# mpeg5/xevd

Measured on AMD Instinct MI355X. Metric: frames/sec (bit-exact YUV) + achieved HBM GB/s, higher is better.
Workload: dtype s16; 1 GPU; cfg4_main_8k_10b_ra; width=7680, height=4320, bit_depth=10, batches_resident=4, residual_pass_ahead=True, parallelism=1 stream on 1 GPU

## Files before the change

include/xevd_hip.h:

```cpp
#ifndef XEVD_HIP_H
#define XEVD_HIP_H

#include <stddef.h>
#include <stdint.h>

#ifdef __cplusplus
extern "C" {
#endif

#define XGPU_OK                    0
#define XGPU_ERR                  (-1)
#define XGPU_ERR_INVALID_ARGUMENT (-101)
#define XGPU_ERR_OUT_OF_MEMORY    (-102)
#define XGPU_ERR_UNSUPPORTED      (-104)
#define XGPU_ERR_UNEXPECTED       (-105)

#define XGPU_MAX_REFS   17
#define XGPU_PAD_L      144
#define XGPU_PAD_C      72

#define XGPU_MODE_INTRA 0
#define XGPU_MODE_INTER 1
#define XGPU_MODE_SKIP  2
#define XGPU_MODE_DIR   3
// ... 298 lines not shown
    const void *d_yuv;
    size_t size;
    int dtype;
    size_t row_pitch;
} xgpu_compare_ref;
typedef struct xgpu_compare_params {
    int crop[4];
    int ssim;
    int block_map;
} xgpu_compare_params;
typedef struct xgpu_compare_result {
    uint64_t n[3];
    uint64_t sse[3];
    uint64_t n_diff[3];
    uint64_t first_diff[3];
    uint32_t max_abs[3];
    uint32_t reserved;
    uint64_t ssim_windows[3];
    int64_t  ssim_q30[3];
} xgpu_compare_result;
size_t xgpu_compare_ref_size(const xgpu_compare_ref *r, int width, int height);
size_t xgpu_compare_map_size(const xgpu_compare_params *p, int width, int height);
int    xgpu_compare_check(const xgpu_compare_ref *r, const xgpu_compare_params *p, int width, int height, int bit_depth);
int    xgpu_pic_compare(xgpu_ctx *ctx, int pic, const xgpu_compare_ref *ref, const xgpu_compare_params *p,
                        xgpu_compare_result *d_result, uint64_t *d_map, size_t map_size, void *stream);
typedef struct xgpu_stats_params {
    int crop[4];
    int hist_bits;
    int pctl_e4[2];
    int light;
    int matrix, full_range, chroma_loc, upsample;
    int transfer;
} xgpu_stats_params;
typedef struct xgpu_stats_result {
    uint64_t n[3], sum[3], sum_sq[3];
    uint32_t min[3], max[3];
    uint32_t pctl[3][2];
    uint64_t light_n;
    double   light_sum, light_mean;
    uint32_t light_max_code, light_pctl_code[2], reserved;
    float    light_max, light_pctl[2], reserved2;
} xgpu_stats_result;
size_t xgpu_stats_hist_size(const xgpu_stats_params *p, int bit_depth);
int    xgpu_stats_check(const xgpu_stats_params *p, int width, int height, int bit_depth);
int    xgpu_stats_lin(int transfer, int bit_depth, float lin[4096]);
int    xgpu_pic_stats(xgpu_ctx *ctx, int pic, const xgpu_stats_params *p, xgpu_stats_result *d_result, uint32_t *d_hist, size_t hist_size, void *stream);
int  xgpu_pic_md5(xgpu_ctx *ctx, int pic, const xgpu_dra_luts *dra, uint8_t digest[3][16]);
int  xgpu_pic_download_padded(xgpu_ctx *ctx, int pic, int16_t *buf_y, int16_t *buf_u, int16_t *buf_v);
int  xgpu_pic_upload_padded(xgpu_ctx *ctx, int pic, const int16_t *buf_y, const int16_t *buf_u, const int16_t *buf_v);

int  xgpu_frame_begin(xgpu_ctx *ctx, const xgpu_frame_params *fp);
int  xgpu_batch_create(xgpu_ctx *ctx, const xgpu_cu_batch *b, xgpu_dbatch **out);
int  xgpu_batch_wait_upload(xgpu_ctx *ctx, xgpu_dbatch *db);
int  xgpu_batch_dmvr_mvs(xgpu_ctx *ctx, xgpu_dbatch *db, int16_t *mv, int n);
int  xgpu_set_builder_threads(xgpu_ctx *ctx, int n);
#define XGPU_BATCH_INFO_COUNT 8
int  xgpu_batch_info(xgpu_ctx *ctx, const xgpu_dbatch *db, int info[XGPU_BATCH_INFO_COUNT]);
void xgpu_batch_destroy(xgpu_ctx *ctx, xgpu_dbatch *db);
int  xgpu_batch_prepare(xgpu_ctx *ctx, xgpu_dbatch *db);
int  xgpu_batch_recon(xgpu_ctx *ctx, xgpu_dbatch *db);
int  xgpu_batch_recon_ahead(xgpu_ctx *ctx, xgpu_dbatch *db, xgpu_dbatch *next);
int  xgpu_deblock(xgpu_ctx *ctx);
int  xgpu_alf(xgpu_ctx *ctx, const xgpu_alf_params *ap);
int  xgpu_pad(xgpu_ctx *ctx);
int  xgpu_frame_end(xgpu_ctx *ctx);

enum { XGPU_K_ITDQ = 0, XGPU_K_INTER = 1, XGPU_K_DBK_V = 2, XGPU_K_DBK_H = 3, XGPU_K_PAD = 4, XGPU_K_INTRA = 5,
       XGPU_K_ALF = 6, XGPU_K_AFFINE = 7, XGPU_K_DMVR = 8, XGPU_K_COUNT = 9 };
int  xgpu_timing_enable(xgpu_ctx *ctx, int on);
int  xgpu_timing_reset(xgpu_ctx *ctx);
int  xgpu_timing_get(xgpu_ctx *ctx, double ms[XGPU_K_COUNT], long long launches[XGPU_K_COUNT]);
int  xgpu_measure_copy_bw(xgpu_ctx *ctx, size_t bytes, int iters, double *gbps);

int xgpu_test_mc_l(xgpu_ctx *ctx, const int16_t *ref_plane, int plane_w, int plane_h, int ref_x, int ref_y,
                   int has_dx, int has_dy, int gmv_x, int gmv_y, int16_t *pred, int w, int h, int bit_depth);
int xgpu_test_mc_c(xgpu_ctx *ctx, const int16_t *ref_plane, int plane_w, int plane_h, int ref_x, int ref_y,
                   int has_dx, int has_dy, int gmv_x, int gmv_y, int16_t *pred, int w, int h, int bit_depth);
int xgpu_test_recon(xgpu_ctx *ctx, const int16_t *coef, const int16_t *pred, int is_coef, int cuw, int cuh, int s_rec, int16_t *rec, int bit_depth);
int xgpu_test_dbk(xgpu_ctx *ctx, int16_t *plane, int pw, int ph, int x, int y, int st, int hor, int bit_depth);
int xgpu_test_dbk_chroma(xgpu_ctx *ctx, int16_t *u, int16_t *v, int pw, int ph, int x, int y, int st_u, int st_v, int hor, int bit_depth);
int xgpu_test_batch_resid(xgpu_ctx *ctx, xgpu_dbatch *db, int16_t *resid);
#define XGPU_TEST_BUILD_DIGESTS 13
int xgpu_test_build_batch(const xgpu_seq_params *sp, const xgpu_cu_batch *b, int threads, uint64_t digest[XGPU_TEST_BUILD_DIGESTS], int info[XGPU_BATCH_INFO_COUNT], double *ms);
int xgpu_test_itdq(xgpu_ctx *ctx, int16_t *coef, int n_blocks, int log2w, int log2h, const uint8_t *qp, int bit_depth);
int xgpu_test_itdq_ex(xgpu_ctx *ctx, int16_t *coef, int n_blocks, int log2w, int log2h, const uint8_t *qp, int bit_depth, int tr_v, int tr_h, int log2s);
int xgpu_test_itdq_pairs(xgpu_ctx *ctx, int16_t *coef, int n_blocks, int log2w, int log2h, const uint8_t *qp, int bit_depth, int tr_v, int tr_h, int log2s);
int xgpu_test_itdq_pairs_mixed(xgpu_ctx *ctx, int16_t *coef, int n_groups, const int32_t *groups, const uint8_t *qp, int bit_depth);
int xgpu_test_scale_taps_device(xgpu_ctx *ctx, int n_plane, int subsampling, int siting_half_luma, int n_dst, int filter, int32_t *first, int32_t *count,
                                int16_t *w, int w_stride);

#ifdef __cplusplus
}
#endif
#endif
```

xevd_amd/abi.py:

```python
import ctypes as C
import os

import numpy as np

HERE = os.path.dirname(os.path.abspath(__file__))
LIB_PATH = os.path.join(HERE, "libxevd_hip.so")

XGPU_MAX_REFS = 17
PAD_L, PAD_C = 144, 72
MODE_INTRA, MODE_INTER, MODE_SKIP, MODE_DIR = 0, 1, 2, 3
K_NAMES = ["itdq", "inter", "dbk_v", "dbk_h", "pad", "intra", "alf", "affine", "dmvr"]
K_COUNT = 9


class SeqParams(C.Structure):
    _fields_ = [
        ("device", C.c_int), ("width", C.c_int), ("height", C.c_int),
        ("bit_depth_luma", C.c_int), ("bit_depth_chroma", C.c_int), ("chroma_format_idc", C.c_int),
        ("log2_ctu", C.c_int), ("tool_iqt", C.c_int), ("tool_admvp", C.c_int), ("tool_addb", C.c_int),
        ("tool_alf", C.c_int), ("max_pics", C.c_int),
        ("chroma_qp_table", C.POINTER(C.c_int8) * 2),
        ("tool_eipd", C.c_int),
    ]

# ... 700 lines not shown
                                              C.c_int, C.c_void_p, C.c_size_t, C.c_void_p]),
    "xgpu_output_scaled_cm_check": (C.c_int, [C.POINTER(OutputFormat), C.POINTER(ScaleParams), C.POINTER(ColourTransform), C.c_int, C.c_int, C.c_int]),
    "xgpu_pic_output_device_scaled_cm": (C.c_int, [C.c_void_p, C.c_int, C.c_void_p, C.POINTER(OutputFormat), C.POINTER(ScaleParams), C.POINTER(ColourTransform),
                                                   C.c_void_p, C.c_size_t, C.c_void_p]),
    "xgpu_pic_output_device_rois_cm": (C.c_int, [C.c_void_p, C.c_int, C.c_void_p, C.POINTER(OutputFormat), C.POINTER(ScaleParams), C.POINTER(RoiParams), C.POINTER(Roi),
                                                 C.c_int, C.POINTER(ColourTransform), C.c_void_p, C.c_size_t, C.c_void_p]),
    "xgpu_output_scaled_lin_check": (C.c_int, [C.POINTER(OutputFormat), C.POINTER(ScaleParams), C.POINTER(ColourTransform), C.c_int, C.c_int, C.c_int]),
    "xgpu_output_rois_lin_check": (C.c_int, [C.POINTER(OutputFormat), C.POINTER(ScaleParams), C.POINTER(RoiParams), C.POINTER(Roi), C.c_int, C.POINTER(ColourTransform),
                                             C.c_int, C.c_int, C.c_int, C.POINTER(C.c_int)]),
    "xgpu_pic_output_device_scaled_lin": (C.c_int, [C.c_void_p, C.c_int, C.c_void_p, C.POINTER(OutputFormat), C.POINTER(ScaleParams), C.POINTER(ColourTransform),
                                                    C.c_void_p, C.c_size_t, C.c_void_p]),
    "xgpu_pic_output_device_rois_lin": (C.c_int, [C.c_void_p, C.c_int, C.c_void_p, C.POINTER(OutputFormat), C.POINTER(ScaleParams), C.POINTER(RoiParams), C.POINTER(Roi),
                                                  C.c_int, C.POINTER(ColourTransform), C.c_void_p, C.c_size_t, C.c_void_p]),
    "xgpu_resample_taps": (C.c_int, [C.c_int] * 6 + [C.POINTER(C.c_int32), C.POINTER(C.c_int32), C.POINTER(C.c_int16), C.c_int]),
    "xgpu_output_resampled_size": (C.c_size_t, [C.POINTER(OutputFormat), C.POINTER(ResampleParams), C.c_int, C.c_int, C.c_int]),
    "xgpu_output_resampled_check": (C.c_int, [C.POINTER(OutputFormat), C.POINTER(ResampleParams), C.c_int, C.c_int, C.c_int]),
    "xgpu_pic_output_device_resampled": (C.c_int, [C.c_void_p, C.c_int, C.c_void_p, C.POINTER(OutputFormat), C.POINTER(ResampleParams), C.c_void_p, C.c_size_t,
                                                   C.c_void_p]),
    "xgpu_output_rois_resampled_check": (C.c_int, [C.POINTER(OutputFormat), C.POINTER(ResampleParams), C.POINTER(RoiParams), C.POINTER(Roi), C.c_int, C.c_int, C.c_int,
                                                   C.c_int, C.POINTER(C.c_int)]),
    "xgpu_output_rois_resampled_size": (C.c_size_t, [C.POINTER(OutputFormat), C.POINTER(ResampleParams), C.POINTER(RoiParams), C.POINTER(Roi), C.c_int, C.c_int, C.c_int,
                                                     C.c_int]),
    "xgpu_pic_output_device_rois_resampled": (C.c_int, [C.c_void_p, C.c_int, C.c_void_p, C.POINTER(OutputFormat), C.POINTER(ResampleParams), C.POINTER(RoiParams),
                                                        C.POINTER(Roi), C.c_int, C.c_void_p, C.c_size_t, C.c_void_p]),
    "xgpu_roi_snap": (C.c_int, [C.c_int, C.c_void_p, C.c_int, C.c_int, C.POINTER(Roi)]),
    "xgpu_output_rois_dev_check": (C.c_int, [C.POINTER(OutputFormat), C.POINTER(ScaleParams), C.POINTER(RoiParams), C.POINTER(RoiBounds)] + [C.c_int] * 5),
    "xgpu_output_rois_dev_size": (C.c_size_t, [C.POINTER(OutputFormat), C.POINTER(ScaleParams), C.POINTER(RoiParams), C.POINTER(RoiBounds)] + [C.c_int] * 5),
    "xgpu_pic_output_device_rois_dev": (C.c_int, [C.c_void_p, C.c_int, C.c_void_p, C.POINTER(OutputFormat), C.POINTER(ScaleParams), C.POINTER(RoiParams),
                                                  C.POINTER(RoiBounds), C.c_int, C.c_void_p, C.c_int, C.c_void_p, C.c_void_p, C.c_void_p, C.c_size_t, C.c_void_p]),
    "xgpu_warp_from_matrix": (C.c_int, [C.POINTER(C.c_double), C.POINTER(WarpMap)]),
    "xgpu_warp_from_rotated_box": (C.c_int, [C.c_double] * 5 + [C.c_int, C.c_int, C.POINTER(WarpMap)]),
    "xgpu_output_warp_check": (C.c_int, [C.POINTER(OutputFormat), C.POINTER(ScaleParams), C.POINTER(WarpParams), C.POINTER(WarpMap), C.c_int, C.c_int, C.c_int, C.c_int,
                                         C.POINTER(C.c_int)]),
    "xgpu_output_warp_size": (C.c_size_t, [C.POINTER(OutputFormat), C.POINTER(ScaleParams), C.POINTER(WarpParams), C.c_int, C.c_int, C.c_int, C.c_int]),
    "xgpu_pic_output_device_warp": (C.c_int, [C.c_void_p, C.c_int, C.c_void_p, C.POINTER(OutputFormat), C.POINTER(ScaleParams), C.POINTER(WarpParams), C.c_void_p,
                                              C.c_int, C.c_int, C.c_void_p, C.c_void_p, C.c_size_t, C.c_void_p]),
    "xgpu_remap_grid_dims": (C.c_int, [C.c_int, C.c_int, C.c_int, C.POINTER(C.c_int), C.POINTER(C.c_int)]),
    "xgpu_remap_grid_size": (C.c_size_t, [C.POINTER(ScaleParams), C.POINTER(RemapParams), C.c_int]),
    "xgpu_output_remap_check": (C.c_int, [C.POINTER(OutputFormat), C.POINTER(ScaleParams), C.POINTER(RemapParams), C.c_int, C.c_int, C.c_int, C.c_int]),
    "xgpu_output_remap_size": (C.c_size_t, [C.POINTER(OutputFormat), C.POINTER(ScaleParams), C.POINTER(RemapParams), C.c_int, C.c_int, C.c_int, C.c_int]),
    "xgpu_remap_from_warp": (C.c_int, [C.POINTER(WarpMap), C.c_int, C.c_int, C.c_int, C.POINTER(C.c_int32)]),
    "xgpu_remap_from_homography": (C.c_int, [C.POINTER(C.c_double), C.c_int, C.c_int, C.c_int, C.POINTER(C.c_int32)]),
    "xgpu_remap_from_lens": (C.c_int, [C.POINTER(RemapLens), C.c_int, C.c_int, C.c_int, C.POINTER(C.c_int32)]),
    "xgpu_pic_output_device_remap": (C.c_int, [C.c_void_p, C.c_int, C.c_void_p, C.POINTER(OutputFormat), C.POINTER(ScaleParams), C.POINTER(RemapParams), C.c_void_p,
                                               C.c_size_t, C.c_int, C.c_void_p, C.c_size_t, C.c_void_p]),
    "xgpu_side_info_size": (C.c_size_t, [C.POINTER(SideFormat), C.c_int, C.c_int]),
    "xgpu_frame_side_info": (C.c_int, [C.c_void_p, C.c_int, C.POINTER(SideFormat), C.c_void_p, C.c_size_t, C.c_void_p]),
    "xgpu_resid_size": (C.c_size_t, [C.POINTER(ResidFormat), C.c_int, C.c_int]),
    "xgpu_batch_residual": (C.c_int, [C.c_void_p, C.c_void_p, C.POINTER(ResidFormat), C.c_void_p, C.c_size_t, C.c_void_p]),
    "xgpu_compare_ref_size": (C.c_size_t, [C.POINTER(CompareRef), C.c_int, C.c_int]),
    "xgpu_compare_map_size": (C.c_size_t, [C.POINTER(CompareParams), C.c_int, C.c_int]),
    "xgpu_compare_check": (C.c_int, [C.POINTER(CompareRef), C.POINTER(CompareParams), C.c_int, C.c_int, C.c_int]),
    "xgpu_pic_compare": (C.c_int, [C.c_void_p, C.c_int, C.POINTER(CompareRef), C.POINTER(CompareParams), C.c_void_p, C.c_void_p, C.c_size_t, C.c_void_p]),
    "xgpu_stats_hist_size": (C.c_size_t, [C.POINTER(StatsParams), C.c_int]),
    "xgpu_stats_check": (C.c_int, [C.POINTER(StatsParams), C.c_int, C.c_int, C.c_int]),
    "xgpu_stats_lin": (C.c_int, [C.c_int, C.c_int, C.POINTER(C.c_float)]),
    "xgpu_pic_stats": (C.c_int, [C.c_void_p, C.c_int, C.POINTER(StatsParams), C.c_void_p, C.c_void_p, C.c_size_t, C.c_void_p]),
    "xgpu_host_alloc": (C.c_int, [C.c_void_p, C.c_size_t, C.POINTER(C.c_void_p)]),
    "xgpu_host_free": (None, [C.c_void_p, C.c_void_p]),
    "xgpu_batch_wait_upload": (C.c_int, [C.c_void_p, C.c_void_p]),
    "xgpu_set_builder_threads": (C.c_int, [C.c_void_p, C.c_int]),
    "xgpu_batch_prepare": (C.c_int, [C.c_void_p, C.c_void_p]),
    "xgpu_batch_info": (C.c_int, [C.c_void_p, C.c_void_p, C.POINTER(C.c_int)]),
    "xgpu_batch_dmvr_mvs": (C.c_int, [C.c_void_p, C.c_void_p, C.c_void_p, C.c_int]),
    "xgpu_pic_download_padded": (C.c_int, [C.c_void_p, C.c_int, C.c_void_p, C.c_void_p, C.c_void_p]),
    "xgpu_pic_upload_padded": (C.c_int, [C.c_void_p, C.c_int, C.c_void_p, C.c_void_p, C.c_void_p]),
    "xgpu_frame_begin": (C.c_int, [C.c_void_p, C.POINTER(FrameParams)]),
    "xgpu_batch_create": (C.c_int, [C.c_void_p, C.POINTER(CuBatch), C.POINTER(C.c_void_p)]),
    "xgpu_batch_destroy": (None, [C.c_void_p, C.c_void_p]),
    "xgpu_batch_recon": (C.c_int, [C.c_void_p, C.c_void_p]),
    "xgpu_batch_recon_ahead": (C.c_int, [C.c_void_p, C.c_void_p, C.c_void_p]),
    "xgpu_deblock": (C.c_int, [C.c_void_p]),
    "xgpu_alf": (C.c_int, [C.c_void_p, C.POINTER(AlfParams)]),
    "xgpu_pad": (C.c_int, [C.c_void_p]),
    "xgpu_frame_end": (C.c_int, [C.c_void_p]),
    "xgpu_timing_enable": (C.c_int, [C.c_void_p, C.c_int]),
    "xgpu_timing_reset": (C.c_int, [C.c_void_p]),
    "xgpu_timing_get": (C.c_int, [C.c_void_p, C.POINTER(C.c_double), C.POINTER(C.c_longlong)]),
    "xgpu_measure_copy_bw": (C.c_int, [C.c_void_p, C.c_size_t, C.c_int, C.POINTER(C.c_double)]),
    "xgpu_test_mc_l": (C.c_int, [C.c_void_p, C.c_void_p] + [C.c_int] * 8 + [C.c_void_p] + [C.c_int] * 3),
    "xgpu_test_mc_c": (C.c_int, [C.c_void_p, C.c_void_p] + [C.c_int] * 8 + [C.c_void_p] + [C.c_int] * 3),
    "xgpu_test_batch_resid": (C.c_int, [C.c_void_p, C.c_void_p, C.c_void_p]),
    "xgpu_test_build_batch": (C.c_int, [C.c_void_p, C.c_void_p, C.c_int, C.POINTER(C.c_uint64), C.POINTER(C.c_int), C.POINTER(C.c_double)]),
    "xgpu_test_recon": (C.c_int, [C.c_void_p, C.c_void_p, C.c_void_p] + [C.c_int] * 4 + [C.c_void_p, C.c_int]),
    "xgpu_test_dbk": (C.c_int, [C.c_void_p, C.c_void_p] + [C.c_int] * 7),
    "xgpu_test_dbk_chroma": (C.c_int, [C.c_void_p, C.c_void_p, C.c_void_p] + [C.c_int] * 8),
    "xgpu_test_itdq": (C.c_int, [C.c_void_p, C.c_void_p, C.c_int, C.c_int, C.c_int, C.c_void_p, C.c_int]),
    "xgpu_test_itdq_ex": (C.c_int, [C.c_void_p, C.c_void_p, C.c_int, C.c_int, C.c_int, C.c_void_p, C.c_int, C.c_int, C.c_int, C.c_int]),
    "xgpu_test_itdq_pairs": (C.c_int, [C.c_void_p, C.c_void_p, C.c_int, C.c_int, C.c_int, C.c_void_p, C.c_int, C.c_int, C.c_int, C.c_int]),
    "xgpu_test_itdq_pairs_mixed": (C.c_int, [C.c_void_p, C.c_void_p, C.c_int, C.c_void_p, C.c_void_p, C.c_int]),
    "xgpu_test_scale_taps_device": (C.c_int, [C.c_void_p] + [C.c_int] * 5 + [C.POINTER(C.c_int32), C.POINTER(C.c_int32), C.POINTER(C.c_int16), C.c_int]),
}

_lib = None


def exported_names():
    return sorted(_EXPORTS)


def _share_torch_hip_runtime():
    import importlib.util
    import sys
    if "torch" in sys.modules:
        return
    spec = importlib.util.find_spec("torch")
    if spec is None or not spec.submodule_search_locations:
        return
    rt = os.path.join(list(spec.submodule_search_locations)[0], "lib", "libamdhip64.so")
    if os.path.exists(rt):
        C.CDLL(rt, mode=C.RTLD_GLOBAL)


def load():
    global _lib
    if _lib is None:
        _share_torch_hip_runtime()
        if not os.path.exists(LIB_PATH):
            raise RuntimeError(
                f"{LIB_PATH} is missing: build it with `python -c 'import __graft_entry__ as g; g.build()'` "
                "(hipcc --offload-arch=gfx950).  xevd_amd has no CPU fallback.")
        lib = C.CDLL(LIB_PATH)
        for name, (res, args) in _EXPORTS.items():
            fn = getattr(lib, name)
            fn.restype, fn.argtypes = res, args
        _lib = lib
    return _lib
```

xevd_amd/csrc/k_alf.hip:

```cpp
#include "xgpu_internal.h"
#include "addb_filter.h"

typedef short v2s __attribute__((ext_vector_type(2)));

#define LROWS 72
#define LSTR  72
#define CROWS 36
#define CSTR  40

struct CtuRect { int x0, y0, cw, ch, aL, aR, aT, aB; int tx0, tx1, ty0, ty1; };

__device__ __forceinline__ void alf_pos(const CtuRect k, int y, int x, int &yy, int &xx)
{
    yy = y; xx = x;
    if (y < k.y0 && !k.aT) yy = 2 * k.y0 - y;
    else if (y >= k.y0 + k.ch && !k.aB) yy = 2 * (k.y0 + k.ch - 1) - y;
    if (yy >= k.y0 && yy < k.y0 + k.ch) {
        if (x < k.x0 && !k.aL) xx = 2 * k.x0 - x;
        else if (x >= k.x0 + k.cw && !k.aR) xx = 2 * (k.x0 + k.cw - 1) - x;
    }
    yy = min(max(yy, k.ty0), k.ty1 - 1); xx = min(max(xx, k.tx0), k.tx1 - 1);
}
__device__ __forceinline__ int alf_fetch(const int16_t *__restrict__ p, int s, const CtuRect k, int y, int x)
{
// ... 25 lines not shown
        } else if (ty0 + r < k.y0 + k.ch + H && tx0 + c4 < k.x0 + k.cw + H) {
#pragma unroll
            for (int e = 0; e < 4; e++) lds[(r + H) * STR + c4 + e + OFF] = (int16_t)alf_fetch(p, s, k, ty0 + r, tx0 + c4 + e);
        }
    }
    constexpr int RING = (T + 2 * H) * (T + 2 * H) - T * T;
    for (int i = t0; i < RING; i += nthr) {
        int r, c;
        if (i < H * (T + 2 * H)) { r = i / (T + 2 * H) - H; c = i % (T + 2 * H) - H; }
        else if (i < 2 * H * (T + 2 * H)) { const int j = i - H * (T + 2 * H); r = T + j / (T + 2 * H); c = j % (T + 2 * H) - H; }
        else { const int j = i - 2 * H * (T + 2 * H); r = j / (2 * H); const int q = j % (2 * H); c = q < H ? q - H : T + q - H; }
        lds[(r + H) * STR + c + OFF] = (int16_t)alf_fetch(p, s, k, ty0 + r, tx0 + c);
    }
}

__device__ __forceinline__ v2s asv(uint32_t x) { return __builtin_bit_cast(v2s, x); }
__device__ __forceinline__ uint32_t asu(v2s x) { return __builtin_bit_cast(uint32_t, x); }
__device__ __forceinline__ v2s vabs(v2s x) { const v2s z = {0, 0}; const v2s n = z - x; return __builtin_elementwise_max(x, n); }
__device__ __forceinline__ int mad_lo(uint32_t ps, int f, int acc) { int r; asm("v_mad_i32_i16 %0, %1, %2, %3" : "=v"(r) : "v"(ps), "v"(f), "v"(acc)); return r; }
__device__ __forceinline__ int mad_hi(uint32_t ps, int f, int acc) { int r; asm("v_mad_i32_i16 %0, %1, %2, %3 op_sel:[1,0,0,0]" : "=v"(r) : "v"(ps), "v"(f), "v"(acc)); return r; }
__device__ __forceinline__ int mad_lo_fh(uint32_t ps, uint32_t f, int acc) { int r; asm("v_mad_i32_i16 %0, %1, %2, %3 op_sel:[0,1,0,0]" : "=v"(r) : "v"(ps), "v"(f), "v"(acc)); return r; }
__device__ __forceinline__ int mad_hi_fh(uint32_t ps, uint32_t f, int acc) { int r; asm("v_mad_i32_i16 %0, %1, %2, %3 op_sel:[1,1,0,0]" : "=v"(r) : "v"(ps), "v"(f), "v"(acc)); return r; }
#define SC_ "s"
__device__ __forceinline__ int smad_lo(uint32_t ps, uint32_t f, int acc) { int r; asm("v_mad_i32_i16 %0, %1, %2, %3" : "=v"(r) : "v"(ps), SC_(f), "v"(acc)); return r; }
__device__ __forceinline__ int smad_hi(uint32_t ps, uint32_t f, int acc) { int r; asm("v_mad_i32_i16 %0, %1, %2, %3 op_sel:[1,0,0,0]" : "=v"(r) : "v"(ps), SC_(f), "v"(acc)); return r; }
__device__ __forceinline__ int smad_lo_fh(uint32_t ps, uint32_t f, int acc) { int r; asm("v_mad_i32_i16 %0, %1, %2, %3 op_sel:[0,1,0,0]" : "=v"(r) : "v"(ps), SC_(f), "v"(acc)); return r; }
__device__ __forceinline__ int smad_hi_fh(uint32_t ps, uint32_t f, int acc) { int r; asm("v_mad_i32_i16 %0, %1, %2, %3 op_sel:[1,1,0,0]" : "=v"(r) : "v"(ps), SC_(f), "v"(acc)); return r; }
__device__ __forceinline__ int dot2s_first(uint32_t f, uint32_t x) { int r; asm("v_dot2_i32_i16 %0, %1, %2, %3" : "=v"(r) : "v"(f), "v"(x), SC_(256)); return r; }
__device__ __forceinline__ int sdot2s(uint32_t f, uint32_t x, int acc) { int r; asm("v_dot2_i32_i16 %0, %1, %2, %3" : "=v"(r) : SC_(f), "v"(x), "v"(acc)); return r; }
__device__ __forceinline__ uint32_t clip_pack(int o0, int o1, int maxv)
{
    int a, b;
    asm("v_med3_i32 %0, %1, 0, %2" : "=v"(a) : "v"(o0 >> 9), SC_(maxv));
    asm("v_med3_i32 %0, %1, 0, %2" : "=v"(b) : "v"(o1 >> 9), SC_(maxv));
    return __builtin_amdgcn_perm((uint32_t)b, (uint32_t)a, 0x05040100u);
}
typedef unsigned short v2us __attribute__((ext_vector_type(2)));
__device__ __forceinline__ uint32_t padd(uint32_t x, uint32_t y) { return __builtin_bit_cast(uint32_t, __builtin_bit_cast(v2us, x) + __builtin_bit_cast(v2us, y)); }
__device__ __forceinline__ uint32_t padd_x(uint32_t x, uint32_t y) { uint32_t r; asm("v_pk_add_u16 %0, %1, %2 op_sel:[0,1] op_sel_hi:[1,0]" : "=v"(r) : "v"(x), "v"(y)); return r; }
__device__ __forceinline__ uint32_t pack_f(int lo, int hi) { return ((uint32_t)lo & 0xFFFFu) | ((uint32_t)hi << 16); }
__device__ __forceinline__ int dot2s(uint32_t f, uint32_t x, int acc) { return __builtin_amdgcn_sdot2(__builtin_bit_cast(v2s, f), __builtin_bit_cast(v2s, x), acc, false); }
__device__ __forceinline__ void lap_pair(const uint32_t up[3], const uint32_t mid[3], const uint32_t dn[3], uint32_t acc[4])
{
    const uint32_t c2 = padd(mid[1], mid[1]);
    const uint32_t l0 = __builtin_amdgcn_alignbit(mid[1], mid[0], 16), r0 = __builtin_amdgcn_alignbit(mid[2], mid[1], 16);
    const uint32_t lu = __builtin_amdgcn_alignbit(up[1], up[0], 16), ru = __builtin_amdgcn_alignbit(up[2], up[1], 16);
    const uint32_t ld = __builtin_amdgcn_alignbit(dn[1], dn[0], 16), rd = __builtin_amdgcn_alignbit(dn[2], dn[1], 16);
    acc[0] = __builtin_amdgcn_sad_u16(c2, padd(up[1], dn[1]), acc[0]);
    acc[1] = __builtin_amdgcn_sad_u16(c2, padd(l0, r0), acc[1]);
    acc[2] = __builtin_amdgcn_sad_u16(c2, padd(lu, rd), acc[2]);
    acc[3] = __builtin_amdgcn_sad_u16(c2, padd(ld, ru), acc[3]);
}

#ifdef XGPU_ALF_TRACE
__device__ unsigned long long g_alf_trace[16];
#define ATR(p) do { if (atr_on) { const unsigned long long now_ = __builtin_amdgcn_s_memtime(); atomicAdd(&g_alf_trace[p], now_ - atr_prev); atr_prev = __builtin_amdgcn_s_memtime(); } } while (0)
extern "C" int xgpu_test_alf_trace(unsigned long long out[16], int reset)
{
    if (hipMemcpyFromSymbol(out, HIP_SYMBOL(g_alf_trace), sizeof(g_alf_trace)) != hipSuccess) return -1;
    if (reset) { static unsigned long long z[16]; if (hipMemcpyToSymbol(HIP_SYMBOL(g_alf_trace), z, sizeof(z)) != hipSuccess) return -1; }
    return 0;
}
#else
#define ATR(p) do { } while (0)
#endif
#ifndef XGPU_ALF_WAVES
#define XGPU_ALF_WAVES 6
#endif
template <bool FUSED, bool PK = false>
__device__ __forceinline__ void alf_kernel(const AlfArgs &a, const AddbArgs *d, const int16_t *__restrict__ sy_, const int16_t *__restrict__ su_,
                                           const int16_t *__restrict__ sv_, int16_t *__restrict__ dy_, int16_t *__restrict__ du_,
                                           int16_t *__restrict__ dv_)
{
    constexpr int RO = FUSED ? 4 : 3, CO = FUSED ? 2 : 4;
    __shared__ __attribute__((aligned(16))) int16_t l_y[LROWS * LSTR];
    __shared__ __attribute__((aligned(16))) int16_t l_c[2][CROWS * CSTR];
    constexpr int LAP_BYTES = 7168;
    static_assert(17 * 17 * 16 <= LAP_BYTES, "the offset-lattice sums fit");
    __shared__ __attribute__((aligned(16))) uint8_t l_lap[LAP_BYTES];
    uint4 (*const l_o)[17] = (uint4 (*)[17])l_lap;
    int16_t (*b_row)[2][64] = (int16_t (*)[2][64])l_y, (*b_col)[2][64] = (int16_t (*)[2][64])(l_y + 3 * 2 * 64);
    static_assert(2 * 3 * 2 * 64 <= LROWS * LSTR, "the border arrays fit into the staged luma tile");

    const int tiles_x = (a.pic_w + 63) >> 6, n_tiles = tiles_x * ((a.pic_h + 63) >> 6);
    const int per_xcd = gridDim.x >> 3, xcd = blockIdx.x & 7, seq = blockIdx.x >> 3;
    const int tile = xcd * per_xcd + (xcd >= 4 ? per_xcd - 1 - seq : seq);
    if (tile >= n_tiles) return;
    const int ty = a.magic_tiles_x ? (int)__umulhi((uint32_t)tile, a.magic_tiles_x) : tile, tx = tile - ty * tiles_x;
    const int tx0 = tx << 6, ty0 = ty << 6;
    const int t = threadIdx.x;
#ifdef XGPU_ALF_TRACE
    unsigned long long atr_prev = __builtin_amdgcn_s_memtime();
    const bool atr_on = (t & 63) == 0 && tile % 61 == 7;
    if (atr_on) atomicAdd(&g_alf_trace[15], 1ull);
#endif
    CtuRect k, kc;
    bool luma_on;
    auto ctu_setup = [&]() {
    const int ctu = 1 << a.log2_ctu;
    k.x0 = tx0 & ~(ctu - 1); k.y0 = ty0 & ~(ctu - 1);
    k.cw = min(ctu, a.pic_w - k.x0); k.ch = min(ctu, a.pic_h - k.y0);
    k.tx0 = 0; k.tx1 = a.pic_w; k.ty0 = 0; k.ty1 = a.pic_h;
    if (a.multi_tile) {
        const int cx = k.x0 >> a.log2_ctu, cy = k.y0 >> a.log2_ctu, h_ctu = (a.pic_h + ctu - 1) >> a.log2_ctu;
        k.tx0 = TileMask::tile_first(a.tiles.vb, cx) << a.log2_ctu; k.tx1 = min(TileMask::tile_end(a.tiles.vb, cx, a.w_ctu) << a.log2_ctu, a.pic_w);
        k.ty0 = TileMask::tile_first(a.tiles.hb, cy) << a.log2_ctu; k.ty1 = min(TileMask::tile_end(a.tiles.hb, cy, h_ctu) << a.log2_ctu, a.pic_h);
    }
    k.aL = a.across_tiles ? k.x0 != 0 : k.x0 != k.tx0; k.aT = a.across_tiles ? k.y0 != 0 : k.y0 != k.ty0;
    k.aR = a.across_tiles ? 1 : (k.x0 + k.cw != k.tx1);
    k.aB = a.across_tiles ? 1 : (k.y0 + k.ch != k.ty1);
    const int ctu_idx = (k.y0 >> a.log2_ctu) * a.w_ctu + (k.x0 >> a.log2_ctu);
    luma_on = a.enable[0] && (a.ctb_in_args ? ((a.ctb_bits[ctu_idx >> 5] >> (ctu_idx & 31)) & 1) != 0 : (a.ctb_flag == nullptr || a.ctb_flag[ctu_idx] != 0));
    kc = k;
    kc.x0 >>= 1; kc.y0 >>= 1; kc.cw >>= 1; kc.ch >>= 1; kc.tx0 >>= 1; kc.tx1 >>= 1; kc.ty0 >>= 1; kc.ty1 >>= 1;
    };
    if (!FUSED) ctu_setup();
    if (!FUSED) {
        if (luma_on) alf_stage<64, 3, LSTR, 4>(l_y, sy_, a.s_l, k, tx0, ty0, t, 256);
        if (a.enable[1]) alf_stage<32, 2, CSTR, 4>(l_c[0], su_, a.s_c, kc, tx0 >> 1, ty0 >> 1, t, 256);
        if (a.enable[2]) alf_stage<32, 2, CSTR, 4>(l_c[1], sv_, a.s_c, kc, tx0 >> 1, ty0 >> 1, t, 256);
        __syncthreads();
    } else {
        const AddbArgs &da = *d;
        uint4 (*s_map)[18] = (uint4 (*)[18])l_lap;
        uint8_t *s_alpha = (uint8_t *)l_lap + 18 * 18 * 16, *s_beta = s_alpha + 52, *s_clip = s_beta + 52, *s_pic = s_clip + 260;
        int8_t *s_cqp = (int8_t *)(s_pic + XGPU_MAX_REFS * 2);
        static_assert(52 + 52 + 260 + XGPU_MAX_REFS * 2 + 192 == ADDB_LDS_TABLE_BYTES, "the LDS tables are AddbArgs.lds_tables");
        constexpr int LIST_OFF = (18 * 18 * 16 + ADDB_LDS_TABLE_BYTES + 3) & ~3;
        uint32_t *s_cnt = (uint32_t *)((uint8_t *)l_lap + LIST_OFF);
        uint32_t (*s_list)[164] = (uint32_t (*)[164])(s_cnt + 2);
        TileMask *s_tm = (TileMask *)((uint8_t *)l_lap + LIST_OFF + 8 + 2 * 164 * 4);
        static_assert(LIST_OFF + 8 + 2 * 164 * 4 + (int)sizeof(TileMask) <= LAP_BYTES, "the deblocking state fits into l_lap");
#define PK2(lo, hi) ((uint32_t)(uint16_t)(lo) | ((uint32_t)(uint16_t)(hi) << 16))
        const bool interior = tx0 > 0 && ty0 > 0 && tx0 + 68 <= a.pic_w && ty0 + 68 <= a.pic_h;
        if (interior) {
            const int wave = __builtin_amdgcn_readfirstlane(t >> 6);
            typedef __attribute__((address_space(3))) char lds_char;
            typedef const __attribute__((address_space(1))) char glb_char;
            {
                const int r0 = (t * 57) >> 9, c0 = t - r0 * 9;
                glb_char *const g0 = (glb_char *)(sy_ + (ty0 - 4) * a.s_l + tx0 - 4);
                lds_char *const d0 = (lds_char *)l_y + wave * 1024;
                const uint32_t rs = (uint32_t)a.s_l << 1;
                const int c1 = c0 + 4 >= 9 ? c0 - 5 : c0 + 4, r1 = r0 + 28 + (c0 + 4 >= 9), c2 = c0 + 8 >= 9 ? c0 - 1 : c0 + 8, r2 = r0 + 56 + (c0 + 8 >= 9);
                __builtin_amdgcn_global_load_lds((glb_char *)(g0 + r0 * rs + c0 * 16), (lds_char *)d0, 16, 0, 0);
                __builtin_amdgcn_global_load_lds((glb_char *)(g0 + r1 * rs + c1 * 16), (lds_char *)(d0 + 4096), 16, 0, 0);
                if (t < 648 - 512) __builtin_amdgcn_global_load_lds((glb_char *)(g0 + r2 * rs + c2 * 16), (lds_char *)(d0 + 8192), 16, 0, 0);
            }
            {
                const uint32_t rs = (uint32_t)a.s_c << 1;
                const uint32_t cbase = (uint32_t)(((ty0 >> 1) - 2) * a.s_c + (tx0 >> 1) - 2) << 1;
                lds_char *const d0 = (lds_char *)&l_c[0][0] + wave * 1024;
#pragma unroll
                for (int it = 0; it < 2; it++) {
                    const int idx = t + 256 * it, pl = idx >= 180, j = idx - 180 * pl, r = (j * 205) >> 10, c = j - r * 5;
                    if (it == 0 || t < 360 - 256)
                        __builtin_amdgcn_global_load_lds((glb_char *)((glb_char *)(pl ? sv_ : su_) + cbase + r * rs + c * 16), (lds_char *)(d0 + 4096 * it), 16, 0, 0);
                }
            }
            {
                glb_char *const g0 = (glb_char *)(da.maps + ((ty0 >> 2) - 1) * da.w_scu + (tx0 >> 2) - 1);
                lds_char *const d0 = (lds_char *)l_lap + wave * 1024;
                const uint32_t rs = (uint32_t)da.w_scu << 4;
#pragma unroll
                for (int it = 0; it < 2; it++) {
                    const int idx = t + 256 * it, r = (idx * 57) >> 10, c = idx - r * 18;
                    if (it == 0 || t < 324 - 256) __builtin_amdgcn_global_load_lds((glb_char *)(g0 + r * rs + c * 16), (lds_char *)(d0 + 4096 * it), 16, 0, 0);
                }
            }
            __builtin_amdgcn_sched_barrier(0);
            {
                static_assert(ADDB_LDS_TABLE_DWORDS + 16 <= 256, "one table dword per thread");
                if (t < ADDB_LDS_TABLE_DWORDS) ((uint32_t *)s_alpha)[t] = da.lds_tables[t];
                else if (t < ADDB_LDS_TABLE_DWORDS + 16) { const int k_ = t - ADDB_LDS_TABLE_DWORDS; ((uint32_t *)s_tm)[k_] = k_ < 8 ? da.no_filter.vb[k_] : da.no_filter.hb[k_ - 8]; }
                if (t < 2) s_cnt[t] = 0;
            }
// ... 347 lines not shown
        if (!a.enable[1 + pl]) {
#pragma unroll
            for (int ii = 0; ii < 2; ii++) {
                const uint32_t w = FUSED ? *(const uint32_t *)(l_c[pl] + ((ly << 1) + ii + 2) * CSTR + (lx << 1) + CO) : *(const uint32_t *)(src + (cy + ii) * a.s_c + cx);
                *(uint32_t *)((char *)dst + (oc0 + ii * sc2)) = w; keep_chroma(ii, w);
            }
            continue;
        }
        uint32_t C[6][3];
#pragma unroll
        for (int i = 0; i < 6; i++) {
            const uint32_t *row = (const uint32_t *)(l_c[pl] + ((ly << 1) + i) * CSTR + (lx << 1) + CO - 2);
            C[i][0] = row[0]; C[i][1] = row[1]; C[i][2] = row[2];
        }
#define PC(i, c) ((((c) + 2) & 1) ? __builtin_amdgcn_alignbit(C[(i) + 2][(((c) + 2) >> 1) + 1], C[(i) + 2][((c) + 2) >> 1], 16) : C[(i) + 2][((c) + 2) >> 1])
        const uint32_t G32 = a.cchroma[0], G54 = a.cchroma[1], G10 = a.cchroma[2], G6 = a.cchroma[3];
        const uint32_t G32v = G32;
#pragma unroll
        for (int ii = 0; ii < 2; ii++) {
            int o[2];
#pragma unroll
            for (int jj = 0; jj < 2; jj++) {
                int acc = sdot2s(G54, padd_x(PC(ii, jj + 1), PC(ii, jj - 2)), dot2s_first(G32v, padd_x(PC(ii + 1, jj - 1), PC(ii - 1, jj))));
                o[jj] = smad_lo(PC(ii, jj), G6, acc);
            }
            const uint32_t p0 = padd(PC(ii + 2, 0), PC(ii - 2, 0)), p1 = padd(PC(ii + 1, 1), PC(ii - 1, -1));
            o[0] = smad_lo_fh(p1, G10, smad_lo(p0, G10, o[0]));
            o[1] = smad_hi_fh(p1, G10, smad_hi(p0, G10, o[1]));
            const uint32_t w = clip_pack(o[0], o[1], maxv);
            *(uint32_t *)((char *)dst + (oc0 + ii * sc2)) = w;
            keep_chroma(ii, w);
        }
#undef PC
    }
    } while (0);

    ATR(11);
    if (!a.pad || !(edge_l || edge_r || edge_t || edge_b)) return;
    __syncthreads();
#pragma unroll
    for (int c = 0; c < 3; c++) {
        const int sh = c ? 1 : 0, pad = c ? XGPU_PAD_C : XGPU_PAD_L, s = c ? a.s_c : a.s_l;
        const int pw = a.pic_w >> sh, ph = a.pic_h >> sh, x0 = tx0 >> sh, y0 = ty0 >> sh, T = 64 >> sh;
        const int cols = min(T, pw - x0), rows = min(T, ph - y0);
        int16_t *pl = c == 0 ? dy_ : (c == 1 ? du_ : dv_);
        const int q = pad >> 2;
#pragma unroll
        for (int side = 0; side < 2; side++) {
            if (side ? !edge_r : !edge_l) continue;
            for (int i = t; i < rows * q; i += 256) {
                const int r = i / q, k = i - r * q;
                const uint32_t v = (uint16_t)b_col[c][side][r] * 0x10001u;
                *(uint2 *)(pl + (y0 + r) * s + (side ? pw : -pad) + 4 * k) = make_uint2(v, v);
            }
        }
#pragma unroll
        for (int side = 0; side < 2; side++) {
            if (side ? !edge_b : !edge_t) continue;
            int16_t *base = pl + (side ? ph : -pad) * s;
            const int cq = cols >> 2;
            for (int i = t; i < pad * cq; i += 256) {
                const int r = i / cq, k = i - r * cq;
                *(uint2 *)(base + r * s + x0 + 4 * k) = *(const uint2 *)&b_row[c][side][4 * k];
            }
#pragma unroll
            for (int cs = 0; cs < 2; cs++) {
                if (cs ? !edge_r : !edge_l) continue;
                const uint32_t v = (uint16_t)b_row[c][side][cs ? cols - 1 : 0] * 0x10001u;
                for (int i = t; i < pad * q; i += 256) {
                    const int r = i / q, k = i - r * q;
                    *(uint2 *)(base + r * s + (cs ? pw : -pad) + 4 * k) = make_uint2(v, v);
                }
            }
        }
    }
}

__global__ __launch_bounds__(256) void k_alf(const AlfArgs a, const int16_t *__restrict__ sy_, const int16_t *__restrict__ su_, const int16_t *__restrict__ sv_,
                                             int16_t *__restrict__ dy_, int16_t *__restrict__ du_, int16_t *__restrict__ dv_)
{
    alf_kernel<false>(a, nullptr, sy_, su_, sv_, dy_, du_, dv_);
}

template <bool PK>
__global__ __launch_bounds__(256) __attribute__((amdgpu_waves_per_eu(XGPU_ALF_WAVES, XGPU_ALF_WAVES))) void k_addb_alf(const AlfArgs a, const AddbArgs d, const int16_t *__restrict__ sy_, const int16_t *__restrict__ su_,
                                                  const int16_t *__restrict__ sv_, int16_t *__restrict__ dy_, int16_t *__restrict__ du_, int16_t *__restrict__ dv_)
{
    alf_kernel<true, PK>(a, &d, sy_, su_, sv_, dy_, du_, dv_);
}

void launch_alf(xgpu_ctx *c, const AlfArgs &a_, const AddbArgs *deblock, const DevPic &src, const DevPic &dst)
{
    AlfArgs a = a_;
    const int tiles = ((a.pic_w + 63) >> 6) * ((a.pic_h + 63) >> 6);
    a.magic_tiles_x = a.pic_w > 64 ? (uint32_t)((1ull << 32) / (uint64_t)((a.pic_w + 63) >> 6)) + 1u : 0u;
    const dim3 grid(((tiles + 7) >> 3) << 3);
    const bool scalar_knob = c->addb_scalar != 0;
    static const int lds_pad = getenv("XEVD_HIP_ALF_LDSPAD") ? atoi(getenv("XEVD_HIP_ALF_LDSPAD")) : 0;
    if (deblock && !scalar_knob && deblock->bd_l <= 10 && deblock->bd_c <= 10) hipLaunchKernelGGL(k_addb_alf<true>, grid, dim3(256), lds_pad, c->stream, a, *deblock, src.y, src.u, src.v, dst.y, dst.u, dst.v);
    else if (deblock) hipLaunchKernelGGL(k_addb_alf<false>, grid, dim3(256), 0, c->stream, a, *deblock, src.y, src.u, src.v, dst.y, dst.u, dst.v);
    else hipLaunchKernelGGL(k_alf, grid, dim3(256), 0, c->stream, a, src.y, src.u, src.v, dst.y, dst.u, dst.v);
}
```

xevd_amd/csrc/k_inter.hip:

```cpp
#include "xgpu_internal.h"

#include <hip/hip_ext.h>
#include <type_traits>
#include "mc_filters.h"

#define LDS_AS __attribute__((address_space(3)))

#define UW_STRIDE 48
#define UI_STRIDE 40
#define UC_STRIDE 24
#define UCW_STRIDE 32
static_assert(UI_STRIDE <= UW_STRIDE && UC_STRIDE <= UCW_STRIDE, "an intermediate row is not longer than the window row it replaces");
#define UT_L_SAMPLES (40 * UW_STRIDE)
#define UT_C_SAMPLES (3 * 64 * 8)
#define UNI_SAMPLES   (UT_L_SAMPLES + UT_C_SAMPLES)
static_assert(2 * 19 * UCW_STRIDE <= UT_C_SAMPLES, "both chroma windows fit");

__device__ __forceinline__ void wave_lds_sync()
{
    __builtin_amdgcn_fence(__ATOMIC_RELEASE, "wavefront");
    __builtin_amdgcn_wave_barrier();
    __builtin_amdgcn_fence(__ATOMIC_ACQUIRE, "wavefront");
}

// ... 548 lines not shown
            }
            TRACE_MARK(tr, 6);
            {
                const uint2 th = s_ctap[cdx ? ((px & 7) << 2) : 32], tv = s_ctap[cdy ? ((py & 7) << 2) : 32];
                const uint32_t c2h[2] = { th.x, th.y }, c2v[2] = { tv.x, tv.y };
                const Regime rg = regime(cdx, cdy, a.bd_c);
                const int mis = ((px >> 3) - 1) & 7, odd = mis & 1;
                const int16_t *const Wu = Wu0 + (mis & ~1), *const Wv = Wu + C_SAMPLES;
                if (cdx) { if (cdy) chroma_tile_filter<true, true, WS_C, true>(Wu, Wv, c2h, c2v, rg, maxc, IC, lane, ou, ov, odd); else chroma_tile_filter<true, false, WS_C, true>(Wu, Wv, c2h, c2v, rg, maxc, IC, lane, ou, ov, odd); }
                else     { if (cdy) chroma_tile_filter<false, true, WS_C, true>(Wu, Wv, c2h, c2v, rg, maxc, IC, lane, ou, ov, odd); else chroma_tile_filter<false, false, WS_C, true>(Wu, Wv, c2h, c2v, rg, maxc, IC, lane, ou, ov, odd); }
            }
            TRACE_MARK(tr, 7);
            if (more) {
                if (REGION) __syncthreads(); else wave_lds_sync();
                request_chroma(1);
            }
            if (nl == 0) {
#pragma unroll
                for (int k = 0; k < 8; k++) pl[k] = o[k];
                pu[0] = ou[0]; pu[1] = ou[1]; pv[0] = ov[0]; pv[1] = ov[1];
            } else {
#pragma unroll
                for (int k = 0; k < 8; k++) pl[k] = avg2(pl[k], o[k]);
                pu[0] = avg2(pu[0], ou[0]); pu[1] = avg2(pu[1], ou[1]);
                pv[0] = avg2(pv[0], ov[0]); pv[1] = avg2(pv[1], ov[1]);
            }
            nl++;
        }
        (void)tid;
    } else {
        TRACE_MARK(tr, 2);
#pragma unroll
        for (int l = 0; l < 2; l++) {
            if (!use[l]) continue;
            const uint4 e0 = s_ref[refis[l] * 2 + l][0], e1 = s_ref[refis[l] * 2 + l][1];
            const gs16 ry_ = (gs16)(((uint64_t)e0.y << 32) | e0.x), ru_ = (gs16)(((uint64_t)e0.w << 32) | e0.z), rv_ = (gs16)(((uint64_t)e1.y << 32) | e1.x);
            const int mvx = mvs[l][0], mvy = mvs[l][1];
            const int px = (x << 2) + mvt[l][0], py = (y << 2) + mvt[l][1];
            const int ldx = (mvx & 3) != 0, ldy = (mvy & 3) != 0;
            const int cdx = (mvx & 7) != 0, cdy = (mvy & 7) != 0;
            uint32_t ch[4], cv[4], o[8], ou[2], ov[2];
            {
                const uint4 th = s_ltap[ldx ? ((px & 3) << 2) : 16], tv = s_ltap[ldy ? ((py & 3) << 2) : 16];
                ch[0] = th.x; ch[1] = th.y; ch[2] = th.z; ch[3] = th.w; cv[0] = tv.x; cv[1] = tv.y; cv[2] = tv.z; cv[3] = tv.w;
                const uint2 cth = s_ctap[cdx ? ((px & 7) << 2) : 32], ctv = s_ctap[cdy ? ((py & 7) << 2) : 32];
                const uint32_t c2h[2] = { cth.x, cth.y }, c2v[2] = { ctv.x, ctv.y };
                const gs16 p = ry_ + ((py >> 2) - 3) * a.s_l + (px >> 2) - 3;
                const int off = ((py >> 3) - 1) * a.s_c + (px >> 3) - 1;
                const Regime rgl = regime(ldx, ldy, a.bd_l), rgc = regime(cdx, cdy, a.bd_c);
                const bool wh = __ballot(ldx) != 0, wvv = __ballot(ldy) != 0;
                const bool cwh = __ballot(cdx) != 0, cwv = __ballot(cdy) != 0;
#define MC_S(H, V) mc_scu_list<H, V>(p, a.s_l, ru_ + off, rv_ + off, a.s_c, ch, cv, rgl, maxl, c2h, c2v, rgc, maxc, cwh, cwv, o, ou, ov, ldx != 0, ldy != 0, cdx != 0, cdy != 0)
                if (wh) { if (wvv) MC_S(true, true); else MC_S(true, false); }
                else    { if (wvv) MC_S(false, true); else MC_S(false, false); }
#undef MC_S
            }
            if (nl == 0) {
#pragma unroll
                for (int k = 0; k < 8; k++) pl[k] = o[k];
                pu[0] = ou[0]; pu[1] = ou[1]; pv[0] = ov[0]; pv[1] = ov[1];
            } else {
#pragma unroll
                for (int k = 0; k < 8; k++) pl[k] = avg2(pl[k], o[k]);
                pu[0] = avg2(pu[0], ou[0]); pu[1] = avg2(pu[1], ou[1]);
                pv[0] = avg2(pv[0], ov[0]); pv[1] = avg2(pv[1], ov[1]);
            }
            nl++;
        }
    }
    TRACE_MARK(tr, 9);
    if (MODE == 0) load_resid();
    if (nl == 0) return false;

    if (cbf & 1) {
#pragma unroll
        for (int k = 0; k < 8; k++) pl[k] = recon2(pl[k], rl[k], maxl);
    }
    if (cbf & 2) { pu[0] = recon2(pu[0], ru[0], maxl); pu[1] = recon2(pu[1], ru[1], maxl); }
    if (cbf & 4) { pv[0] = recon2(pv[0], rv[0], maxl); pv[1] = recon2(pv[1], rv[1], maxl); }

    return true;
}

__device__ __forceinline__ int xcd_slice(int block, int grid) { return (block & 7) * (grid >> 3) + (block >> 3); }

__device__ __forceinline__ void store_scu(const InterArgs &a, int sx, int sy, const uint32_t pl[8], const uint32_t pu[2], const uint32_t pv[2])
{
    const int x = sx << 2, y = sy << 2;
    int16_t *dy = a.cur_y + y * a.s_l + x;
#pragma unroll
    for (int k = 0; k < 4; k++) *(uint2 *)(dy + k * a.s_l) = make_uint2(pl[k * 2], pl[k * 2 + 1]);
    const int coff = (y >> 1) * a.s_c + (x >> 1);
    *(uint32_t *)(a.cur_u + coff) = pu[0];
    *(uint32_t *)(a.cur_u + coff + a.s_c) = pu[1];
    *(uint32_t *)(a.cur_v + coff) = pv[0];
    *(uint32_t *)(a.cur_v + coff + a.s_c) = pv[1];
}
#define ARG_REFS(a)  ((const uint4 (*)[2])&(a).refp[0][0])
#define ARG_LTAPS(a) ((const uint4 *)&k_luma_taps[(a).admvp][0][0])
#define ARG_CTAPS(a) ((const uint2 *)&k_chroma_taps[(a).admvp][0][0])
static_assert(sizeof(RefEntry) == 32, "a reference entry is two 16-byte halves");
static_assert(XGPU_INTER_STRIP == 16, "the strip arithmetic below shifts by four");

struct SplitTables { uint4 ref[XGPU_MAX_REFS * 2][2]; uint4 ltap[17]; uint2 ctap[33]; uint2 pad; };

__device__ __forceinline__ void inter_fused_body(const InterArgs &a)
{
    __shared__ __attribute__((aligned(16))) int16_t s_win[REG_SAMPLES];
    static_assert(4 * UNI_SAMPLES <= REG_SAMPLES, "the four waves' tile blocks fit into the region block");
    __shared__ SplitTables s_tab[4];
    const int idx = xcd_slice(blockIdx.x, gridDim.x);
    if (idx >= a.n_work) return;
    const int t = threadIdx.x, lane = t & 63, wave = __builtin_amdgcn_readfirstlane(t >> 6);
#ifdef XGPU_INTER_TRACE
    InterTrace tr = { __builtin_amdgcn_s_memtime(), 0, lane == 0 && (idx % 61) == 7 };
#endif
    int rx, ry;
    if (idx < a.full_entries) {
        const int s = (int)__umulhi((uint32_t)idx, a.magic_strip), r = idx - s * a.strip_entries;
        ry = r >> 4; rx = (s << 4) + (r & 15);
    } else {
        const int r = idx - a.full_entries;
        ry = a.magic_last ? (int)__umulhi((uint32_t)r, a.magic_last) : r; rx = (a.regions_x & ~15) + r - ry * (a.regions_x & 15);
    }
    const int sx = (rx << 4) + ((wave & 1) << 3) + (lane & 7), sy = (ry << 4) + ((wave >> 1) << 3) + (lane >> 3);
    const uint32_t kinds = a.work[idx];
    const uint4 *const item = (const uint4 *)&a.items[idx * 4 + wave];
    const uint4 e = item[0], i0 = item[1], i1 = item[2];
    const uint32_t own = (sx < (a.pic_w >> 2) && sy < (a.pic_h >> 2)) ? a.owner[sy * a.w_scu + sx] : OWNER_NONE;
    const LaneMap fm0 = { 0, 0 };
    uint32_t pl[8], pu[2], pv[2];
    if (kinds == XGPU_WORK_REGION) {
#ifdef XGPU_INTER_TRACE
        tr.role = 0;
        if (e.y == 0xFFFFFFFFu) tr.on = false;
        if (tr.on) atomicAdd(&g_inter_trace[0][15], 1ull);
        TRACE_MARK(tr, 0);
#endif
        const RegionMap rmap = region_map(t);
        if (inter_tile<2>(a, i0, i1, true, sx, sy, lane, s_win, fm0, ARG_REFS(a), ARG_LTAPS(a), ARG_CTAPS(a), pl, pu, pv, &rmap, wave, e.y TRACE_PASS)) store_scu(a, sx, sy, pl, pu, pv);
        TRACE_MARK(tr, 10);
        return;
    }
    const uint32_t kind = (kinds >> (2 * wave)) & 3u;
    if (kind == 1) {
#ifdef XGPU_INTER_TRACE
        tr.role = 1;
        if (e.y == 0xFFFFFFFFu) tr.on = false;
        if (tr.on) atomicAdd(&g_inter_trace[1][15], 1ull);
        TRACE_MARK(tr, 0);
#endif
        LaneMap fm;
        {
            const int row0 = (lane * 171) >> 10, k = lane - row0 * 6;
            fm.gy = row0 * a.s_l + 8 * k; fm.ly = row0 * UW_STRIDE + 8 * k;
        }
        if (inter_tile<1>(a, i0, i1, true, sx, sy, lane, s_win + wave * UNI_SAMPLES, fm, ARG_REFS(a), ARG_LTAPS(a), ARG_CTAPS(a), pl, pu, pv, nullptr, 0, e.y TRACE_PASS)) store_scu(a, sx, sy, pl, pu, pv);
        TRACE_MARK(tr, 10);
    } else if (kind == 2) {
#ifdef XGPU_INTER_TRACE
        tr.role = 2;
        if (tr.on) atomicAdd(&g_inter_trace[2][15], 1ull);
        TRACE_MARK(tr, 0);
#endif
        SplitTables &tb = s_tab[wave];
        static_assert(XGPU_MAX_REFS * 4 == 68, "lanes 0..63 and 0..3 of the second round take the reference entries' halves");
        const uint4 tab0 = ((const uint4 *)&a.refp[0][0])[lane];
        uint4 tab1 = make_uint4(0, 0, 0, 0);
        if (lane < 4) tab1 = ((const uint4 *)&a.refp[0][0])[64 + lane];
        else if (lane < 4 + 17) tab1 = *(const uint4 *)k_luma_taps[a.admvp][lane - 4];
        else if (lane < 4 + 17 + 33) { const uint2 v = *(const uint2 *)k_chroma_taps[a.admvp][lane - 21]; tab1.x = v.x; tab1.y = v.y; }
        const bool ok = own < (uint32_t)a.n_cu;
        uint4 c0 = make_uint4(0, 0, 0, 0), c1 = c0;
        if (ok) { c0 = ((const uint4 *)&a.cus[own])[0]; c1 = ((const uint4 *)&a.cus[own])[1]; }
        tb.ref[lane >> 1][lane & 1] = tab0;
        if (lane < 4) tb.ref[32 + (lane >> 1)][lane & 1] = tab1;
        else if (lane < 4 + 17) tb.ltap[lane - 4] = tab1;
        else if (lane < 4 + 17 + 33) tb.ctap[lane - 21] = make_uint2(tab1.x, tab1.y);
        wave_lds_sync();
        TRACE_MARK(tr, 1);
        if (inter_tile<0>(a, c0, c1, ok, sx, sy, lane, nullptr, fm0, tb.ref, tb.ltap, tb.ctap, pl, pu, pv, nullptr, 0, own TRACE_PASS)) store_scu(a, sx, sy, pl, pu, pv);
        TRACE_MARK(tr, 10);
    }
}
__global__ __launch_bounds__(256) void k_inter(const InterArgs a) { inter_fused_body(a); }

void launch_inter(xgpu_ctx *c, const InterArgs &a)
{
    if (!a.n_work) return;
    const dim3 grid((unsigned)(((a.n_work + 7) >> 3) << 3));
    hipLaunchKernelGGL(k_inter, grid, dim3(256), 0, c->stream, a);
}

__global__ void k_test_mc(const int16_t *plane, int stride, int ref_x, int ref_y, int has_dx, int has_dy, int gmv_x, int gmv_y,
                          int16_t *pred, int w, int h, int bd, int luma, int admvp)
{
    const int bs = luma ? 4 : 2;
    const int nbx = w / bs, nby = h / bs;
    const int i = blockIdx.x * blockDim.x + threadIdx.x;
    if (i >= nbx * nby) return;
    const int bx = (i % nbx) * bs, by = (i / nbx) * bs;
    const int maxv = (1 << bd) - 1;
    const int16_t *ref = plane + ref_y * stride + ref_x;
    if (luma) {
        const uint32_t *th = k_luma_taps[admvp][has_dx ? (gmv_x & 15) : 16], *tv = k_luma_taps[admvp][has_dy ? (gmv_y & 15) : 16];
        uint32_t ch[4] = { th[0], th[1], th[2], th[3] }, cv[4] = { tv[0], tv[1], tv[2], tv[3] }, o[8];
        const gs16 p = (gs16)ref + ((gmv_y >> 4) - 3 + by) * stride + (gmv_x >> 4) - 3 + bx;
        if (has_dx) { if (has_dy) mc_luma_4x4<true, true>(p, stride, ch, cv, regime(has_dx, has_dy, bd), maxv, o); else mc_luma_4x4<true, false>(p, stride, ch, cv, regime(has_dx, has_dy, bd), maxv, o); }
        else        { if (has_dy) mc_luma_4x4<false, true>(p, stride, ch, cv, regime(has_dx, has_dy, bd), maxv, o); else mc_luma_4x4<false, false>(p, stride, ch, cv, regime(has_dx, has_dy, bd), maxv, o); }
        for (int r = 0; r < 4; r++) {
            *(uint32_t *)(pred + (by + r) * w + bx) = o[r * 2];
            *(uint32_t *)(pred + (by + r) * w + bx + 2) = o[r * 2 + 1];
        }
    } else {
        const uint32_t *th = k_chroma_taps[admvp][has_dx ? (gmv_x & 31) : 32], *tv = k_chroma_taps[admvp][has_dy ? (gmv_y & 31) : 32];
        uint32_t ch[2] = { th[0], th[1] }, cv[2] = { tv[0], tv[1] }, o[2];
        const gs16 p = (gs16)ref + ((gmv_y >> 5) - 1 + by) * stride + (gmv_x >> 5) - 1 + bx;
        if (has_dx) { if (has_dy) mc_chroma_2x2<true, true>(p, stride, ch, cv, regime(has_dx, has_dy, bd), maxv, o); else mc_chroma_2x2<true, false>(p, stride, ch, cv, regime(has_dx, has_dy, bd), maxv, o); }
        else        { if (has_dy) mc_chroma_2x2<false, true>(p, stride, ch, cv, regime(has_dx, has_dy, bd), maxv, o); else mc_chroma_2x2<false, false>(p, stride, ch, cv, regime(has_dx, has_dy, bd), maxv, o); }
        *(uint32_t *)(pred + by * w + bx) = o[0];
        *(uint32_t *)(pred + (by + 1) * w + bx) = o[1];
    }
}

void launch_test_mc(xgpu_ctx *c, const int16_t *plane, int stride, int ref_x, int ref_y, int has_dx, int has_dy,
                    int gmv_x, int gmv_y, int16_t *pred, int w, int h, int bd, int luma)
{
    const int bs = luma ? 4 : 2;
    const int n = (w / bs) * (h / bs);
    hipLaunchKernelGGL(k_test_mc, dim3((n + 63) / 64), dim3(64), 0, c->stream, plane, stride, ref_x, ref_y, has_dx, has_dy,
                       gmv_x, gmv_y, pred, w, h, bd, luma, c->sp.tool_admvp);
}

__global__ void k_test_recon(const int16_t *coef, const int16_t *pred, int is_coef, int cuw, int cuh, int16_t *rec, int s_rec, int bd)
{
    const int i = blockIdx.x * blockDim.x + threadIdx.x, pw = cuw >> 1;
    if (i >= pw * cuh) return;
    const int y = i / pw, x = (i - y * pw) * 2;
    const uint32_t p = *(const uint32_t *)(pred + y * cuw + x);
    const uint32_t r = recon2(p, is_coef ? *(const uint32_t *)(coef + y * cuw + x) : 0u, (1 << bd) - 1);
    rec[y * s_rec + x] = (int16_t)(r & 0xFFFF); rec[y * s_rec + x + 1] = (int16_t)(r >> 16);
}
void launch_test_recon(xgpu_ctx *c, const int16_t *coef, const int16_t *pred, int is_coef, int cuw, int cuh, int16_t *rec, int s_rec, int bd)
{
    const int n = (cuw >> 1) * cuh;
    hipLaunchKernelGGL(k_test_recon, dim3((n + 63) / 64), dim3(64), 0, c->stream, coef, pred, is_coef, cuw, cuh, rec, s_rec, bd);
}
```

xevd_amd/csrc/xgpu_api.hip:

```cpp
#include "xgpu_host.h"

static const int8_t k_chroma_qp_main[58] = { 0, 1, 2, 3, 4, 5, 6, 7, 8, 9, 10, 11, 12, 13, 14, 15, 16, 17, 18, 19, 20, 21, 22, 23, 24, 25, 26, 27, 28, 29,
    29, 30, 31, 32, 33, 34, 35, 36, 37, 37, 38, 39, 40, 40, 41, 42, 43, 44, 45, 46, 47, 48, 49, 50, 51, 52, 53, 54 };
static const int8_t k_chroma_qp_base[58] = {
     0,  1,  2,  3,  4,  5,  6,  7,  8,  9, 10, 11, 12, 13, 14, 15, 16, 17, 18, 19,
    20, 21, 22, 23, 24, 25, 26, 27, 28, 29, 29, 29, 30, 31, 32, 32, 33, 33, 34, 34,
    35, 35, 36, 36, 36, 37, 37, 37, 38, 38, 39, 39, 40, 40, 40, 41, 41, 41 };


const char *xgpu_version(void) { return "xevd_amd 0.1 (gfx950)"; }
const char *xgpu_last_error(const xgpu_ctx *c) { return c ? c->err : "null ctx"; }

void time_begin(xgpu_ctx *c, int k, hipEvent_t *a, hipEvent_t *b)
{
    if (!c->timing) return;
    auto get = [&]() {
        hipEvent_t e;
        if (!c->ev_pool.empty()) { e = c->ev_pool.back(); c->ev_pool.pop_back(); }
        else (void)hipEventCreate(&e);
        return e;
    };
    *a = get(); *b = get();
    (void)hipEventRecord(*a, c->stream);
    (void)k;
// ... 6 lines not shown
}
int xgpu_timing_enable(xgpu_ctx *c, int on) { ARGCHK(c, c != NULL); c->timing = on; return XGPU_OK; }
int xgpu_timing_reset(xgpu_ctx *c)
{
    ARGCHK(c, c != NULL);
    HIPCHK(c, hipStreamSynchronize(c->stream));
    for (auto &e : c->ev_pending) { c->ev_pool.push_back(e.a); c->ev_pool.push_back(e.b); }
    c->ev_pending.clear();
    memset(c->t_ms, 0, sizeof(c->t_ms));
    memset(c->t_n, 0, sizeof(c->t_n));
    return XGPU_OK;
}
int xgpu_timing_get(xgpu_ctx *c, double ms[XGPU_K_COUNT], long long n[XGPU_K_COUNT])
{
    ARGCHK(c, c != NULL);
    HIPCHK(c, hipStreamSynchronize(c->stream));
    for (auto &e : c->ev_pending) {
        float t = 0;
        HIPCHK(c, hipEventElapsedTime(&t, e.a, e.b));
        c->t_ms[e.k] += t; c->t_n[e.k]++;
        c->ev_pool.push_back(e.a); c->ev_pool.push_back(e.b);
    }
    c->ev_pending.clear();
    for (int i = 0; i < XGPU_K_COUNT; i++) { ms[i] = c->t_ms[i]; n[i] = c->t_n[i]; }
    return XGPU_OK;
}

static void init_transform_tables(xgpu_ctx *c)
{
    static int tm[5460];
    int o = 0;
    for (int l = 1; l <= 6; l++) {
        const int N = 1 << l;
        for (int k = 0; k < N; k++)
            for (int n = 0; n < N; n++) {
                const double v = k == 0 ? 64.0 : 64.0 * sqrt(2.0) * cos((2 * n + 1) * k * 3.14159265358979323846 / (2.0 * N));
                tm[o++] = (int)(v >= 0 ? floor(v + 0.5) : -floor(-v + 0.5));
            }
    }
    static int16_t ats[2 * 1360];
    for (int t = 0; t < 2; t++) {
        int q = t * 1360;
        for (int l = 2; l <= 5; l++) {
            const int N = 1 << l;
            const double sc = sqrt((double)N) * 64;
            int16_t m[32 * 32];
            for (int k = 0; k < N; k++)
                for (int n = 0; n < N; n++) {
                    const double v = t == 0 ? sin(3.14159265358979323846 * (k + 0.5) * (n + 1) / (N + 0.5)) * sqrt(2.0 / (N + 0.5))
                                            : cos(3.14159265358979323846 * (k + 0.5) * (n + 0.5) / (N + 0.5)) * sqrt(2.0 / (N + 0.5));
                    m[k * N + n] = (int16_t)(sc * v + (v > 0 ? 0.5 : -0.5));
                }
            if (N == 4) {
                const int a = m[0], b = m[1], cc = m[2], d = m[3];
                const int e7[16] = { a, b, cc, b + a,  cc, cc, 0, -cc,  a + b, -a, -cc, b,  b, -(b + a), cc, -a };
                const int e8[16] = { d + cc, b, cc, d,  b, 0, -b, -b,  cc, -b, -d, d + cc,  d, -b, d + cc, -cc };
                for (int i = 0; i < 16; i++) m[i] = (int16_t)(t == 0 ? e7[i] : e8[i]);
            }
            for (int i = 0; i < N * N; i++) ats[q++] = m[i];
        }
    }
    upload_transform_tables(tm, ats, c->stream);
}

int xgpu_open(const xgpu_seq_params *sp, xgpu_ctx **out)
{
    if (!sp || !out) return XGPU_ERR_INVALID_ARGUMENT;
    *out = NULL;
    if (sp->chroma_format_idc != 1) return XGPU_ERR_UNSUPPORTED;
    if (sp->width <= 0 || sp->height <= 0 || (sp->width & 7) || (sp->height & 7)) return XGPU_ERR_INVALID_ARGUMENT;
    if (sp->bit_depth_luma < 8 || sp->bit_depth_luma > 12 || sp->bit_depth_chroma < 8 || sp->bit_depth_chroma > 12) return XGPU_ERR_UNSUPPORTED;
    if (sp->log2_ctu < 5 || sp->log2_ctu > 7) return XGPU_ERR_INVALID_ARGUMENT;
    int ndev = 0;
    if (hipGetDeviceCount(&ndev) != hipSuccess || ndev <= 0 || sp->device < 0 || sp->device >= ndev) return XGPU_ERR_UNEXPECTED;

    xgpu_ctx *c = new xgpu_ctx();
    c->sp = *sp;
    c->sp.chroma_qp_table[0] = c->sp.chroma_qp_table[1] = NULL;
    c->builder_threads = 1;
    c->err[0] = 0; c->timing = 0; c->have_frame = 0; c->side_pic = -1; c->d_maps = NULL; c->d_dra = NULL; c->d_cm = NULL; c->cm_tab = NULL; c->d_ctb_flag = NULL; c->stream = 0; c->up_stream = 0; c->down_stream = 0; c->side_stream = 0; c->after_inter = 0; c->have_after_inter = 0; c->where = 0; c->addb_pending = 0;
    c->fork_ev = c->join_ev = 0;
    c->itdq_pair_min = getenv("XEVD_HIP_ITDQ_PAIR_MIN") ? std::max(1, atoi(getenv("XEVD_HIP_ITDQ_PAIR_MIN"))) : 4096;
    c->intra_small_min = getenv("XEVD_HIP_INTRA_SMALL_MIN") ? std::max(1, atoi(getenv("XEVD_HIP_INTRA_SMALL_MIN"))) : 2048;
    c->addb_scalar = getenv("XEVD_HIP_ADDB_SCALAR") != NULL;
    c->dmvr_scalar = getenv("XEVD_HIP_DMVR_SCALAR") != NULL;
    c->split_addb_alf = getenv("XEVD_HIP_SPLIT_ADDB_ALF") != NULL;
    for (int i = 0; i < 2; i++) { c->d_out[i] = NULL; c->out_caps[i] = 0; c->out_ready[i] = c->out_done[i] = 0; c->out_busy[i] = 0; }
    c->d_md5 = NULL; c->md5_ready = 0;
    c->odev_ev[0] = c->odev_ev[1] = 0;
    c->sc_tab = NULL; c->sc_tab_cap = 0; c->sc_mid = NULL; c->sc_mid_cap = 0; c->cmp_part = NULL; c->cmp_part_cap = 0; c->stats_blk = NULL; c->stats_lin_tc = c->stats_lin_bd = -1;
    c->roi_blk = NULL; c->roi_blk_cap = 0;
    c->rs_blk = NULL; c->rs_blk_cap = 0; c->rs_key[0] = -1; c->rs_capy = c->rs_capc = 0;
    c->lad_blk = NULL; c->lad_blk_cap = 0; c->lad_cap = 0;
    for (int i = 0; i < 6; i++) c->sc_key[i] = -1;
    c->out_next = 0;
    memset(c->t_ms, 0, sizeof(c->t_ms)); memset(c->t_n, 0, sizeof(c->t_n));
    const int boff = 6 * (sp->bit_depth_chroma - 8);
    for (int t = 0; t < 2; t++)
        for (int q = -boff; q <= 57; q++)
            c->chroma_qp[t][q + boff] = sp->chroma_qp_table[t] ? sp->chroma_qp_table[t][q + boff] : (int8_t)(q < 0 ? q : (sp->tool_iqt ? k_chroma_qp_main[q] : k_chroma_qp_base[q]));

    auto fail = [&](int code) { xgpu_close(c); return code; };
    if (hipSetDevice(sp->device) != hipSuccess) return fail(XGPU_ERR_UNEXPECTED);
    static const bool blocking = getenv("XEVD_HIP_BLOCKING_SYNC") != NULL && atoi(getenv("XEVD_HIP_BLOCKING_SYNC")) != 0;
    if (blocking) (void)hipSetDeviceFlags(hipDeviceScheduleBlockingSync);
    const unsigned ev_flags = hipEventDisableTiming | (blocking ? hipEventBlockingSync : 0);
    {
        static std::atomic<int> n_ctx(0);
        static const bool no_rot = getenv("XEVD_HIP_NO_QUEUE_ROTATION") != NULL;
        const bool swap = !no_rot && (n_ctx.fetch_add(1) & 1);
        hipStream_t *const order[4] = { swap ? &c->side_stream : &c->stream, &c->up_stream, &c->down_stream, swap ? &c->stream : &c->side_stream };
        for (int i = 0; i < 4; i++)
            if (hipStreamCreateWithFlags(order[i], hipStreamNonBlocking) != hipSuccess) return fail(XGPU_ERR_UNEXPECTED);
    }
    if (hipEventCreateWithFlags(&c->after_inter, hipEventDisableTiming) != hipSuccess) return fail(XGPU_ERR_UNEXPECTED);
    if (hipEventCreateWithFlags(&c->fork_ev, hipEventDisableTiming) != hipSuccess || hipEventCreateWithFlags(&c->join_ev, hipEventDisableTiming) != hipSuccess) return fail(XGPU_ERR_UNEXPECTED);
    for (int i = 0; i < 2; i++)
        if (hipEventCreateWithFlags(&c->out_ready[i], hipEventDisableTiming) != hipSuccess || hipEventCreateWithFlags(&c->out_done[i], ev_flags) != hipSuccess)
            return fail(XGPU_ERR_UNEXPECTED);

    ctx_geometry(c);

    if (hipMalloc((void **)&c->d_maps, sizeof(ScuRec) * (size_t)c->w_scu * c->h_scu) != hipSuccess) return fail(XGPU_ERR_OUT_OF_MEMORY);
    if (hipMemsetAsync(c->d_maps, 0, sizeof(ScuRec) * (size_t)c->w_scu * c->h_scu, c->stream) != hipSuccess) return fail(XGPU_ERR_UNEXPECTED);
    if (hipMalloc((void **)&c->d_ctb_flag, (size_t)c->w_ctu * c->h_ctu + 16) != hipSuccess) return fail(XGPU_ERR_OUT_OF_MEMORY);
    init_transform_tables(c);
    c->pics.resize(1 + std::max(1, std::min(sp->max_pics, 34)));
    for (auto &p : c->pics) { p.base = NULL; p.used = 0; }
    {
        DevPic &p = c->pics[0];
        if (hipMalloc((void **)&p.base, c->pic_elems * sizeof(int16_t)) != hipSuccess) return fail(XGPU_ERR_OUT_OF_MEMORY);
        (void)hipMemsetAsync(p.base, 0, c->pic_elems * sizeof(int16_t), c->stream);
        p.s_l = c->s_l; p.s_c = c->s_c; p.used = 1;
        p.y = p.base + (size_t)XGPU_PAD_L * c->s_l + XGPU_MARGIN_L;
        p.u = p.base + c->off_u + (size_t)XGPU_PAD_C * c->s_c + XGPU_MARGIN_C;
        p.v = p.base + c->off_v + (size_t)XGPU_PAD_C * c->s_c + XGPU_MARGIN_C;
    }
    if (hipStreamSynchronize(c->stream) != hipSuccess) return fail(XGPU_ERR_UNEXPECTED);
    *out = c;
    return XGPU_OK;
}

void xgpu_close(xgpu_ctx *c)
{
    if (!c) return;
    (void)hipSetDevice(c->sp.device);
    if (c->stream) (void)hipStreamSynchronize(c->stream);
    if (c->up_stream) (void)hipStreamSynchronize(c->up_stream);
    if (c->down_stream) (void)hipStreamSynchronize(c->down_stream);
    if (c->side_stream) (void)hipStreamSynchronize(c->side_stream);
    for (auto &p : c->pics) if (p.base) (void)hipFree(p.base);
    if (c->d_maps) (void)hipFree(c->d_maps);
    for (BatchBlock &k : c->pool) block_free(k);
    for (auto &h : c->pinned) (void)hipHostFree(h.p);
    c->pinned.clear();
    c->pool.clear();
    if (c->d_md5) (void)hipFree(c->d_md5);
    if (c->md5_ready) (void)hipEventDestroy(c->md5_ready);
    for (int i = 0; i < 2; i++) if (c->odev_ev[i]) (void)hipEventDestroy(c->odev_ev[i]);
    for (int i = 0; i < 2; i++) { if (c->d_out[i]) (void)hipFree(c->d_out[i]); if (c->out_ready[i]) (void)hipEventDestroy(c->out_ready[i]); if (c->out_done[i]) (void)hipEventDestroy(c->out_done[i]); }
    if (c->d_dra) (void)hipFree(c->d_dra);
    if (c->d_cm) (void)hipFree(c->d_cm);
    delete c->cm_tab;
    if (c->sc_tab) (void)hipFree(c->sc_tab);
    if (c->sc_mid) (void)hipFree(c->sc_mid);
    if (c->cmp_part) (void)hipFree(c->cmp_part);
// ... 241 lines not shown
```

xevd_amd/csrc/xgpu_builder.hip:

```cpp
#include <chrono>
#include "xgpu_host.h"
#include "affine_model.h"

namespace {
enum Seg { SEG_CUS, SEG_CTU, SEG_TBS, SEG_WAVES, SEG_INTRA, SEG_DEPS, SEG_AFF, SEG_CPMV, SEG_DMVR, SEG_OWNER, SEG_IITEM, SEG_IWORK, SEG_COEF, SEG_RESID, SEG_DONE, SEG_DMV, SEG_COUNT };
struct StageLayout {
    size_t off[SEG_COUNT], alloc[SEG_COUNT], payload[SEG_COUNT], stage_bytes, d_need;
    template <class T> T *at(void *base, Seg s) const { return (T *)((uint8_t *)base + off[s]); }
};
struct SegSize { Seg seg; size_t elem, count, min_count; };
template <size_t N> void stage_layout(StageLayout &L, const SegSize (&rows)[N])
{
    static_assert(N == SEG_COUNT, "one row per segment");
    size_t o = 0;
    for (const SegSize &r : rows) {
        L.off[r.seg] = o; L.payload[r.seg] = r.elem * r.count; L.alloc[r.seg] = r.elem * std::max(r.count, r.min_count);
        if (r.seg == SEG_COEF) L.stage_bytes = o + L.alloc[r.seg];
        o += (L.alloc[r.seg] + 255) / 256 * 256;
    }
    L.d_need = o;
}
enum { NCLS = 64 * 9 };
inline int ats_inter_of(const xgpu_cu_batch *b, int i) { return (b->ats_inter && b->pred_mode[i] != XGPU_MODE_INTRA && b->pred_mode[i] != XGPU_MODE_IBC) ? b->ats_inter[i] : 0; }
inline int tr_code(const xgpu_cu_batch *b, int i, int k)
{
    if (k != 0) return 0;
    if (const int ai = ats_inter_of(b, i)) {
        if (b->log2w[i] > 5 || b->log2h[i] > 5) return 0;
        const int idx = ai & 15, pos = ai >> 4, hor = idx == 2 || idx == 4;
        const int tv = hor ? (pos == 0 ? TR_DCT8 : TR_DST7) : TR_DST7, th = hor ? TR_DST7 : (pos == 0 ? TR_DCT8 : TR_DST7);
        return tv * 3 + th;
    }
    if (!b->ats || !(b->ats[i] & 1) || b->pred_mode[i] != XGPU_MODE_INTRA) return 0;
    const int tv = (b->ats[i] >> 1) & 1 ? TR_DCT8 : TR_DST7, th = (b->ats[i] >> 2) & 1 ? TR_DCT8 : TR_DST7;
    return tv * 3 + th;
}
template <class F> inline size_t for_each_tb(const xgpu_cu_batch *b, int i, F &&f)
{
    int bw = b->log2w[i], bh = b->log2h[i]; const int idx = ats_inter_of(b, i) & 15;
    if (idx == 1 || idx == 3) bw -= idx == 3 ? 2 : 1;
    if (idx == 2 || idx == 4) bh -= idx == 4 ? 2 : 1;
    const int nsx = b->log2w[i] > 6 ? 2 : 1, nsy = b->log2h[i] > 6 ? 2 : 1;
    size_t ext = 0;
    for (int k = 0; k < 3; k++) {
        if (!((b->cbf[i] >> k) & 1)) continue;
        const int cl = k ? bw - 1 : bw, ch = k ? bh - 1 : bh;
        const int tw = std::min(bw, 6) - (k ? 1 : 0), th = std::min(bh, 6) - (k ? 1 : 0), cls = tr_code(b, i, k) * 64 + tw * 8 + th;
        for (int sb = 0; sb < 4; sb++) {
            if ((sb & 1) >= nsx || (sb >> 1) >= nsy) continue;
            if (nsx * nsy > 1 && b->cbf_sub && !((b->cbf_sub[i] >> (4 * k + sb)) & 1)) continue;
            f(k, sb, cls, tw, th, cl, (uint32_t)ext);
        }
        ext += (size_t)1 << (cl + ch);
    }
    return ext;
}
inline int closing_chroma_cu(const xgpu_cu_batch *b, int i) { int j = i + 1; while (j < b->n_cu && b->tree[j] != 2) j++; return j; }
inline bool dmvr_cand(const xgpu_cu_batch *b, int i)
{
    return b->dmvr && b->dmvr[i] && b->pred_mode[i] != XGPU_MODE_INTRA && b->pred_mode[i] != XGPU_MODE_IBC && !(b->affine && b->affine[i]) &&
           b->refi[i * 2] >= 0 && b->refi[i * 2 + 1] >= 0 && b->log2w[i] >= 3 && b->log2h[i] >= 3;
}
inline bool affine_is_eif(const xgpu_cu_batch *b, int i)
{
    const bool use[2] = { b->refi[i * 2] >= 0, b->refi[i * 2 + 1] >= 0 };
    AffModel md[2];
    for (int l = 0; l < 2; l++) md[l] = aff_model(b->affine_mv + (size_t)i * 12 + l * 6, b->log2w[i], b->log2h[i], b->affine[i]);
    int sw, sh; bool mb;
    aff_subblock(md, use, b->log2w[i], b->log2h[i], sw, sh, mb);
    return sw < 8 || sh < 8;
}
struct Part { int cls[NCLS]; int n_aff, n_eif, n_sub, n_dmvr; std::vector<uint32_t> nodes; };
struct Build {
    xgpu_ctx *c; const xgpu_cu_batch *b; BuilderScratch &S; int n, nthr;
    std::vector<Part> parts;
    int cls_count[NCLS], cls_first[NCLS], n_tb, n_waves, n_aff, n_aff_eif, n_aff_sub, n_dmvr;
    template <class F> void run_parts(F fn) { S.pool.run(nthr, [&](int k) { fn(k, (int)((long long)n * k / nthr), (int)((long long)n * (k + 1) / nthr)); }); }
    void copy_sliced(void *dst, const void *src, size_t bytes)
    {
        S.pool.run(nthr, [&](int k) { const size_t a0 = bytes * (size_t)k / nthr & ~(size_t)63, a1 = k + 1 == nthr ? bytes : (bytes * (size_t)(k + 1) / nthr & ~(size_t)63);
                                      memcpy((uint8_t *)dst + a0, (const uint8_t *)src + a0, a1 - a0); });
    }
#define CUCHK(cond) do { if (!(cond)) return #cond; } while (0)
    const char *validate_and_count(int i0, int i1, Part &P)
    {
        for (int i = i0; i < i1; i++) {
            const int lw = b->log2w[i], lh = b->log2h[i];
            CUCHK(lw >= 2 && lw <= 7 && lh >= 2 && lh <= 7 && lw <= c->sp.log2_ctu && lh <= c->sp.log2_ctu);
// ... 6 lines not shown
                    const int j = closing_chroma_cu(b, i);
                    CUCHK(j < n && b->x[j] <= b->x[i] && b->y[j] <= b->y[i] && b->x[i] + (1 << lw) <= b->x[j] + (1 << b->log2w[j]) && b->y[i] + (1 << lh) <= b->y[j] + (1 << b->log2h[j]));
                }
            }
            if (b->pred_mode[i] == XGPU_MODE_IBC) {
                const int bvx = b->mv[i * 4], bvy = b->mv[i * 4 + 1];
                CUCHK(b->x[i] + (bvx & ~1) >= 0 && b->y[i] + (bvy & ~1) >= 0 && b->x[i] + bvx + (1 << lw) <= c->sp.width && b->y[i] + bvy + (1 << lh) <= c->sp.height);
                CUCHK(!(b->affine && b->affine[i]));
            } else if (b->pred_mode[i] != XGPU_MODE_INTRA) CUCHK(b->refi[i * 2] < XGPU_MAX_REFS && b->refi[i * 2 + 1] < XGPU_MAX_REFS);
            CUCHK(b->qp[i * 3] < 96 && b->qp[i * 3 + 1] < 96 && b->qp[i * 3 + 2] < 96);
            if (const int ai = ats_inter_of(b, i)) {
                const int idx = ai & 15, pos = ai >> 4;
                CUCHK(idx >= 1 && idx <= 4 && pos <= 1 && lw <= 6 && lh <= 6);
                CUCHK(((idx == 1 || idx == 3) ? lw : lh) >= (idx >= 3 ? 4 : 3));
            }
            if (b->affine && b->affine[i]) {
                CUCHK(b->affine_mv != NULL && (b->affine[i] == 2 || b->affine[i] == 3) && b->pred_mode[i] != XGPU_MODE_INTRA);
                CUCHK(lw >= 3 && lh >= 3 && (b->refi[i * 2] >= 0 || b->refi[i * 2 + 1] >= 0));
                P.n_aff++;
                if (affine_is_eif(b, i)) P.n_eif += ((1 << lw) + 15) / 16 * (((1 << lh) + 15) / 16);
                else                     P.n_sub += ((1 << lw) + 31) / 32 * (((1 << lh) + 31) / 32);
            }
            if (dmvr_cand(b, i)) P.n_dmvr += (lw > 4 ? 1 << (lw - 4) : 1) * (lh > 4 ? 1 << (lh - 4) : 1);
            const char *bad = nullptr;
            const size_t need = for_each_tb(b, i, [&](int, int, int cls, int tw, int th, int, uint32_t) {
                if (cls < 64 || (tw >= 2 && tw <= 5 && th >= 2 && th <= 5)) P.cls[cls]++;
                else bad = "tr_code(i, k) == 0 || (tw >= 2 && tw <= 5 && th >= 2 && th <= 5)";
            });
            if (bad) return bad;
            CUCHK((size_t)b->coef_off[i] + need <= b->n_coef);
            if (plan_is_node(b, (uint32_t)i)) P.nodes.push_back((uint32_t)i);
        }
        return nullptr;
    }
#undef CUCHK
    int pass1()
    {
        parts.resize((size_t)nthr);
        std::vector<const char *> bad((size_t)nthr, nullptr);
        run_parts([&](int k, int i0, int i1) { bad[(size_t)k] = validate_and_count(i0, i1, parts[(size_t)k]); });
        for (const char *m : bad)
            if (m) { snprintf(c->err, sizeof(c->err), "%s: invalid argument: %s", __FILE__, m); return XGPU_ERR_INVALID_ARGUMENT; }
        for (const Part &P : parts) { for (int k = 0; k < NCLS; k++) cls_count[k] += P.cls[k]; n_aff += P.n_aff; n_aff_eif += P.n_eif; n_aff_sub += P.n_sub; n_dmvr += P.n_dmvr; }
        for (int k = 0; k < NCLS; k++) {
            cls_first[k] = n_tb; n_tb += cls_count[k];
            if (cls_count[k]) { const int per = itdq_group_size((k & 63) >> 3, k & 7); n_waves += (cls_count[k] + per - 1) / per; }
        }
        return XGPU_OK;
    }
    void paint_owner_map()
    {
        std::vector<uint32_t> &own = S.own; own.resize((size_t)c->w_scu * c->h_scu);
        size_t covered = 0;
        for (int i = 0; i < n; i++) if (!(b->tree && b->tree[i] == 2)) covered += (size_t)1 << (b->log2w[i] + b->log2h[i] - 4);
        if (covered != own.size()) std::fill(own.begin(), own.end(), 0xFFFFFFFFu);
        uint32_t *const own_p = own.data();
        run_parts([&, own_p](int, int i0, int i1) {
            for (int i = i0; i < i1; i++) {
                if (b->tree && b->tree[i] == 2) continue;
                const int ws = (1 << b->log2w[i]) >> 2, hh = (1 << b->log2h[i]) >> 2;
                uint32_t *o = own_p + (size_t)(b->y[i] >> 2) * c->w_scu + (b->x[i] >> 2);
                for (int r = 0; r < hh; r++, o += c->w_scu) std::fill_n(o, ws, (uint32_t)i);
            }
        });
    }
    void inter_work_lists()
    {
        std::vector<uint32_t> &inter_items = S.inter_items, &inter_work = S.inter_work;
        const int tiles_x = (c->sp.width + 31) >> 5, tiles_y = (c->sp.height + 31) >> 5, full_x = c->sp.width >> 5, full_y = c->sp.height >> 5;
        S.tile_cu.assign((size_t)tiles_x * tiles_y, 0xFFFFFFFFu);
        S.tile_any.assign((size_t)tiles_x * tiles_y, 0);
        uint32_t *const tcu = S.tile_cu.data(); uint8_t *const tany = S.tile_any.data();
        run_parts([&, tcu, tany](int, int i0, int i1) {
            for (int i = i0; i < i1; i++) {
                if (b->tree && b->tree[i] == 2) continue;
                const int x0 = b->x[i], y0 = b->y[i], x1 = x0 + (1 << b->log2w[i]), y1 = y0 + (1 << b->log2h[i]);
                for (int ty = y0 >> 5; ty <= (y1 - 1) >> 5; ty++)
                    for (int tx = x0 >> 5; tx <= (x1 - 1) >> 5; tx++) {
                        if (tx < full_x && ty < full_y && (tx << 5) >= x0 && (tx << 5) + 32 <= x1 && (ty << 5) >= y0 && (ty << 5) + 32 <= y1) tcu[(size_t)ty * tiles_x + tx] = (uint32_t)i;
                        else __atomic_store_n(&tany[(size_t)ty * tiles_x + tx], (uint8_t)1, __ATOMIC_RELAXED);
                    }
            }
        });
        inter_items.clear(); inter_work.clear();
        const int regions_x = (c->sp.width + 63) >> 6, regions_y = (c->sp.height + 63) >> 6;
        for (int s0 = 0; s0 < regions_x; s0 += XGPU_INTER_STRIP)
            for (int ry = 0; ry < regions_y; ry++)
                for (int rx = s0; rx < std::min(s0 + XGPU_INTER_STRIP, regions_x); rx++) {
                    const int tx = rx * 2, ty = ry * 2;
                    const bool whole = tx + 1 < tiles_x && ty + 1 < tiles_y;
                    const uint32_t o = tcu[(size_t)ty * tiles_x + tx];
                    if (whole && o != 0xFFFFFFFFu && tcu[(size_t)ty * tiles_x + tx + 1] == o && tcu[(size_t)(ty + 1) * tiles_x + tx] == o && tcu[(size_t)(ty + 1) * tiles_x + tx + 1] == o) {
                        inter_work.push_back(XGPU_WORK_REGION);
                        for (int q = 0; q < 4; q++) inter_items.push_back(o);
                        continue;
                    }
                    uint32_t kinds = 0;
                    for (int q = 0; q < 4; q++) {
                        const int ux = tx + (q & 1), uy = ty + (q >> 1);
                        uint32_t oq = 0xFFFFFFFFu;
                        if (ux < tiles_x && uy < tiles_y) {
                            oq = tcu[(size_t)uy * tiles_x + ux];
                            if (oq != 0xFFFFFFFFu) kinds |= 1u << (2 * q);
                            else if (tany[(size_t)uy * tiles_x + ux]) kinds |= 2u << (2 * q);
                        }
                        inter_items.push_back(oq);
                    }
                    inter_work.push_back(kinds);
                }
    }
    bool probe_order_rl()
    {
        if (c->sp.tool_addb) return false;
        std::atomic<int> found(0); const uint32_t *const own_p = S.own.data();
        run_parts([&, own_p](int, int i0, int i1) {
            for (int i = i0; i < i1 && !found.load(std::memory_order_relaxed); i++) {
                const int xr = b->x[i] + (1 << b->log2w[i]);
                if (xr < c->sp.width && own_p[(size_t)(b->y[i] >> 2) * c->w_scu + (xr >> 2)] < (uint32_t)i) found.store(1, std::memory_order_relaxed);
            }
        });
        return found.load() != 0;
    }
    bool intra_plan()
    {
        S.nodes.clear(); S.plan.reset();
        for (const Part &P : parts) S.nodes.insert(S.nodes.end(), P.nodes.begin(), P.nodes.end());
        return S.nodes.empty() || build_intra_plan(c, b, S, S.own.data(), nthr);
    }
    int acquire_block(xgpu_dbatch *db, const StageLayout &L, bool &coef_pinned)
    {
        int best = -1;
        {
            std::lock_guard<std::mutex> g(c->pool_mu);
            for (const auto &h : c->pinned)
                if ((const uint8_t *)b->coef >= h.p && (const uint8_t *)(b->coef + b->n_coef) <= h.p + h.n) coef_pinned = b->n_coef != 0;
            for (size_t k = 0; k < c->pool.size(); k++)
                if (c->pool[k].d_cap >= L.d_need && c->pool[k].h_cap >= L.stage_bytes && (best < 0 || c->pool[k].d_cap < c->pool[best].d_cap)) best = (int)k;
            if (best >= 0) { db->blk = c->pool[best]; c->pool.erase(c->pool.begin() + best); }
        }
        if (db->host_only) {
            memset(&db->blk, 0, sizeof(db->blk));
            if (S.host_stage.size() < L.stage_bytes) S.host_stage.resize(L.stage_bytes);
            db->blk.h_stage = S.host_stage.data(); db->blk.h_cap = L.stage_bytes;
        } else if (best >= 0) {
            if (hipEventSynchronize(db->blk.uploaded) != hipSuccess) return XGPU_ERR_UNEXPECTED;
            if (hipStreamWaitEvent(c->up_stream, db->blk.done, 0) != hipSuccess) return XGPU_ERR_UNEXPECTED;
        } else {
            memset(&db->blk, 0, sizeof(db->blk));
            const size_t d_cap = L.d_need + L.d_need / 4, h_cap = L.stage_bytes + L.stage_bytes / 4;
            if (hipMalloc((void **)&db->blk.d_base, d_cap) != hipSuccess) return XGPU_ERR_OUT_OF_MEMORY;
            if (hipHostMalloc(&db->blk.h_stage, h_cap, hipHostMallocDefault) != hipSuccess) return XGPU_ERR_OUT_OF_MEMORY;
            db->blk.d_cap = d_cap; db->blk.h_cap = h_cap;
            static const bool blocking = getenv("XEVD_HIP_BLOCKING_SYNC") != NULL && atoi(getenv("XEVD_HIP_BLOCKING_SYNC")) != 0;
            if (hipEventCreateWithFlags(&db->blk.uploaded, hipEventDisableTiming | (blocking ? hipEventBlockingSync : 0)) != hipSuccess) return XGPU_ERR_UNEXPECTED;
            if (hipEventCreateWithFlags(&db->blk.done, hipEventDisableTiming) != hipSuccess) return XGPU_ERR_UNEXPECTED;
            if (hipEventCreateWithFlags(&db->blk.itdq_done, hipEventDisableTiming) != hipSuccess) return XGPU_ERR_UNEXPECTED;
        }
        if (db->n_chroma_cus) {
            const size_t nb = sizeof(uint32_t) * (size_t)db->n_chroma_cus;
            if (db->blk.chroma_cap < nb) {
                if (db->blk.d_chroma) (void)hipFree(db->blk.d_chroma);
                db->blk.d_chroma = NULL; db->blk.chroma_cap = 0;
                if (hipMalloc((void **)&db->blk.d_chroma, nb + nb / 4) != hipSuccess) return XGPU_ERR_OUT_OF_MEMORY;
                db->blk.chroma_cap = nb + nb / 4;
            }
            db->d_chroma_cus = db->blk.d_chroma;
        }
        return XGPU_OK;
    }
    void fill_records(const StageLayout &L, void *hs)
    {
        CuRec *const cus = L.at<CuRec>(hs, SEG_CUS); TbRec *const tbs = L.at<TbRec>(hs, SEG_TBS); int16_t *const cpmv = L.at<int16_t>(hs, SEG_CPMV);
        AffItem *const aff_items = L.at<AffItem>(hs, SEG_AFF); DmvrItem *const dmvr_items = L.at<DmvrItem>(hs, SEG_DMVR);
        const int bdoff = 6 * (c->sp.bit_depth_luma - 8);
        run_parts([&](int part, int i0, int i1) {
        int cls_fill[NCLS]; memcpy(cls_fill, cls_first, sizeof(cls_fill));
        int aff_fill = 0, eif_fill = 0, sub_fill = n_aff_eif, dmvr_fill = 0;
        for (int q = 0; q < part; q++) {
            const Part &P = parts[(size_t)q];
            for (int k = 0; k < NCLS; k++) cls_fill[k] += P.cls[k];
            aff_fill += P.n_aff; eif_fill += P.n_eif; sub_fill += P.n_sub; dmvr_fill += P.n_dmvr;
        }
        for (int i = i0; i < i1; i++) {
            CuRec &r = cus[i]; memset(&r, 0, sizeof(r));
            if (b->affine && b->affine[i]) {
                r.affine = b->affine[i];
                memcpy(cpmv + (size_t)aff_fill * 12, b->affine_mv + (size_t)i * 12, sizeof(int16_t) * 12);
                const bool eif = affine_is_eif(b, i);
                const int step = eif ? 16 : 32;
                for (int ty = 0; ty < (1 << b->log2h[i]); ty += step)
                    for (int tx = 0; tx < (1 << b->log2w[i]); tx += step) {
                        AffItem &it = aff_items[eif ? eif_fill++ : sub_fill++];
                        it.cu = (uint32_t)i; it.aff = (uint32_t)aff_fill; it.tx = (uint16_t)tx; it.ty = (uint16_t)ty; it.pad = 0;
                    }
                aff_fill++;
            }
            r.x = b->x[i]; r.y = b->y[i]; r.log2w = b->log2w[i]; r.log2h = b->log2h[i];
            r.pred_mode = b->pred_mode[i]; r.cbf = b->cbf[i] & 7;
            if (b->tree && b->tree[i] == 1) {
                const int j = closing_chroma_cu(b, i);
                if (b->x[i] != b->x[j]) r.pred_mode |= CU_NOCH_L;
                if (b->y[i] != b->y[j]) r.pred_mode |= CU_NOCH_T;
            }
            r.refi[0] = b->refi[i * 2]; r.refi[1] = b->refi[i * 2 + 1];
            r.qp_map = (uint8_t)((b->qp[i * 3] - bdoff) & 0x7F);
            r.map_cbf = (uint8_t)((r.cbf & 1) && (!(r.log2w > 6 || r.log2h > 6) || !b->cbf_sub || (b->cbf_sub[i] & 1)));
            r.coef_off = b->coef_off[i];
            memcpy(r.mv, &b->mv[i * 4], sizeof(r.mv));
            r.qp[0] = b->qp[i * 3]; r.qp[1] = b->qp[i * 3 + 1]; r.qp[2] = b->qp[i * 3 + 2];
            if (b->ipm) { r.ipm[0] = b->ipm[i * 2]; r.ipm[1] = b->ipm[i * 2 + 1]; }
            r.ats_inter = (uint8_t)ats_inter_of(b, i);
            if (dmvr_cand(b, i)) {
                r.dmvr = 1;
                const int dxs = std::min(1 << b->log2w[i], 16), dys = std::min(1 << b->log2h[i], 16);
                for (int sy = 0; sy < (1 << b->log2h[i]); sy += dys)
                    for (int sx = 0; sx < (1 << b->log2w[i]); sx += dxs) {
                        DmvrItem &it = dmvr_items[dmvr_fill++];
                        it.cu = (uint32_t)i; it.sx = (uint8_t)(sx >> 2); it.sy = (uint8_t)(sy >> 2); it.pad = 0;
                    }
            }
            for_each_tb(b, i, [&](int k, int sb, int cls, int tw, int th, int cl, uint32_t comp_off) {
                TbRec &t = tbs[cls_fill[cls]++];
                t.off = r.coef_off + comp_off + ((uint32_t)(sb >> 1) << (th + cl)) + ((uint32_t)(sb & 1) << tw);
                t.log2w = (uint8_t)tw; t.log2h = (uint8_t)th; t.qp = r.qp[k]; t.log2s = (uint8_t)cl;
            });
        }
        });
    }
    void fill_work_items(TbWave *wv)
    {
        int w = 0;
        for (int sz = 12; sz >= 2; sz--)
        for (int k = 0; k < NCLS; k++) {
            if (!cls_count[k] || ((k & 63) >> 3) + (k & 7) != sz) continue;
            const int per = itdq_group_size((k & 63) >> 3, k & 7);
            for (int f = 0; f < cls_count[k]; f += per) {
                wv[w].first = cls_first[k] + f; wv[w].count = (uint16_t)std::min(per, cls_count[k] - f);
                wv[w].log2w = (uint8_t)((k & 63) >> 3); wv[w].log2h = (uint8_t)(k & 7);
                wv[w].tr_v = (uint8_t)((k >> 6) / 3); wv[w].tr_h = (uint8_t)((k >> 6) % 3); wv[w].pad[0] = wv[w].pad[1] = 0; w++;
            }
        }
    }
    void fill_items_and_copies(const StageLayout &L, void *hs)
    {
        memcpy(L.at<uint8_t>(hs, SEG_CTU), b->ctu_cu_start, L.payload[SEG_CTU]);
        InterItem *const it = L.at<InterItem>(hs, SEG_IITEM); const CuRec *const cus = L.at<CuRec>(hs, SEG_CUS);
        const uint32_t *const ii = S.inter_items.data(); const size_t n_items = S.inter_items.size();
        S.pool.run(nthr, [&, it, ii](int part) {
            for (size_t k = n_items * (size_t)part / nthr; k < n_items * (size_t)(part + 1) / nthr; k++) {
                if (ii[k] == 0xFFFFFFFFu) memset(&it[k], 0, sizeof(InterItem));
                else { it[k].pos = 0; it[k].cu = ii[k]; it[k].pad[0] = it[k].pad[1] = 0; it[k].rec = cus[ii[k]]; }
            }
        });
        if (L.payload[SEG_IWORK]) memcpy(L.at<uint8_t>(hs, SEG_IWORK), S.inter_work.data(), L.payload[SEG_IWORK]);
        if (L.payload[SEG_COEF]) copy_sliced(L.at<uint8_t>(hs, SEG_COEF), b->coef, L.payload[SEG_COEF]);
        if (L.payload[SEG_INTRA]) memcpy(L.at<uint8_t>(hs, SEG_INTRA), S.plan.recs.data(), L.payload[SEG_INTRA]);
        if (L.payload[SEG_DEPS]) memcpy(L.at<uint8_t>(hs, SEG_DEPS), S.plan.deps.data(), L.payload[SEG_DEPS]);
    }
    hipError_t upload(xgpu_dbatch *db, const StageLayout &L, bool coef_pinned)
    {
        uint8_t *const dbase = db->blk.d_base;
        hipError_t e = hipMemcpyAsync(dbase, db->h_stage, coef_pinned ? L.off[SEG_COEF] : L.stage_bytes, hipMemcpyHostToDevice, c->up_stream);
        if (e == hipSuccess && coef_pinned) e = hipMemcpyAsync(dbase + L.off[SEG_COEF], b->coef, sizeof(int16_t) * b->n_coef, hipMemcpyHostToDevice, c->up_stream);
        if (e == hipSuccess && db->n_chroma_cus) e = hipMemcpyAsync(db->d_chroma_cus, db->h_chroma_cus, sizeof(uint32_t) * (size_t)db->n_chroma_cus, hipMemcpyHostToDevice, c->up_stream);
        if (e == hipSuccess) e = hipMemsetAsync(db->d_intra_done, 0, L.alloc[SEG_DONE], c->up_stream);
        if (e == hipSuccess) e = hipMemsetAsync(db->d_resid, 0, L.alloc[SEG_RESID], c->up_stream);
        if (e == hipSuccess) e = hipEventRecord(db->blk.uploaded, c->up_stream);
        return e;
    }
};
void batch_info_fill(const xgpu_dbatch *db, int info[XGPU_BATCH_INFO_COUNT])
{
    info[0] = db->n_cu; info[1] = db->n_tb; info[2] = db->n_waves; info[3] = db->n_intra; info[4] = db->n_intra_l1; info[5] = db->n_levels; info[6] = db->n_dmvr; info[7] = db->n_aff_eif + db->n_aff_sub;
}
int batch_build(xgpu_ctx *c, const xgpu_cu_batch *b, xgpu_dbatch **out, bool host_only, StageLayout *layout)
{
    ARGCHK(c, c != NULL); ARGCHK(c, b != NULL && out != NULL);
    *out = NULL;
    ARGCHK(c, b->n_cu >= 0 && b->n_ctu == c->w_ctu * c->h_ctu);
    ARGCHK(c, b->n_cu == 0 || (b->x && b->y && b->log2w && b->log2h && b->pred_mode && b->refi && b->mv && b->qp && b->cbf && b->coef_off));
    ARGCHK(c, b->ctu_cu_start != NULL && (b->n_coef == 0 || b->coef != NULL));
    ARGCHK(c, b->htdf_slice_qp >= 0 && b->htdf_slice_qp <= 51);
    ARGCHK(c, b->ctu_cu_start[0] == 0 && b->ctu_cu_start[b->n_ctu] == (uint32_t)b->n_cu);
    for (int k = 0; k < b->n_ctu; k++) ARGCHK(c, b->ctu_cu_start[k] <= b->ctu_cu_start[k + 1]);
    TileMask tmask; ARGCHK(c, tile_mask(c, b->tiles, tmask));
    if (!host_only) HIPCHK(c, hipSetDevice(c->sp.device));
    static const bool bt_on = getenv("XEVD_HIP_BUILD_TRACE") != NULL;
    auto bt_t0 = std::chrono::steady_clock::now();
    auto BT = [&](const char *what) { if (bt_on) { const auto t = std::chrono::steady_clock::now(); fprintf(stderr, "  batch build: %-14s %.2f ms\n", what, std::chrono::duration<double, std::milli>(t - bt_t0).count()); bt_t0 = t; } };
    static thread_local BuilderScratch scratch;
    const int n = b->n_cu;
    Build B = { c, b, scratch, n, std::max(1, std::min(c->builder_threads, std::max(1, n / 4096))) };
    BuilderScratch &S = B.S; const IntraPlan &plan = S.plan;
    if (const int rc = B.pass1()) return rc;
    BT("pass 1");
    B.paint_owner_map();
    BT("owner map");
    B.inter_work_lists();
    BT("inter lists");
    const bool order_rl = B.probe_order_rl();
    ARGCHK(c, B.intra_plan());
    const int n_intra = (int)plan.recs.size(), n_deps = (int)plan.deps.size();
    BT("intra plan");
    xgpu_dbatch *db = new xgpu_dbatch();
    memset(db, 0, sizeof(*db)); db->host_only = host_only ? 1 : 0;
    db->n_cu = n; db->n_ctu = b->n_ctu; db->n_tb = B.n_tb; db->n_waves = B.n_waves; db->n_coef = b->n_coef; db->n_intra = n_intra; db->n_intra_deps = n_deps; db->n_levels = plan.n_levels; db->n_intra_l1 = plan.n_level1; db->n_intra_l1_small = plan.n_level1_small; db->n_intra_heads = plan.n_heads; db->n_aff_eif = B.n_aff_eif; db->n_aff_sub = B.n_aff_sub; db->n_dmvr = B.n_dmvr; db->has_ibc = plan.has_ibc ? 1 : 0; db->has_htdf = plan.has_htdf ? 1 : 0; db->has_right = plan.has_right ? 1 : 0; db->order_rl = order_rl ? 1 : 0;
    db->tile_starts = tmask; db->tiles_across = b->tiles ? (b->tiles->loop_filter_across_tiles ? 1 : 0) : 1; db->n_inter_work = (int)S.inter_work.size();
    const SegSize rows[] = { { SEG_CUS, sizeof(CuRec), (size_t)n, 1 }, { SEG_CTU, sizeof(uint32_t), (size_t)b->n_ctu + 1, 1 }, { SEG_TBS, sizeof(TbRec), (size_t)B.n_tb, 1 }, { SEG_WAVES, sizeof(TbWave), (size_t)B.n_waves, 1 },
        { SEG_INTRA, sizeof(IntraRec), (size_t)n_intra, 1 }, { SEG_DEPS, sizeof(uint32_t), (size_t)n_deps, 1 }, { SEG_AFF, sizeof(AffItem), (size_t)(B.n_aff_eif + B.n_aff_sub), 1 }, { SEG_CPMV, sizeof(int16_t) * 12, (size_t)B.n_aff, 1 },
        { SEG_DMVR, sizeof(DmvrItem), (size_t)B.n_dmvr, 1 }, { SEG_OWNER, sizeof(uint32_t), (size_t)c->w_scu * c->h_scu, 0 }, { SEG_IITEM, sizeof(InterItem), S.inter_items.size(), 1 }, { SEG_IWORK, sizeof(uint32_t), S.inter_work.size(), 1 },
        { SEG_COEF, sizeof(int16_t), b->n_coef, 8 }, { SEG_RESID, sizeof(int16_t), b->n_coef, 8 }, { SEG_DONE, sizeof(uint32_t), (size_t)n_intra + 1, 1 }, { SEG_DMV, sizeof(int16_t) * 4, (size_t)B.n_dmvr, 1 } };
    StageLayout L; stage_layout(L, rows); db->stage_bytes = L.stage_bytes;
    auto fail = [&](int code) { xgpu_batch_destroy(c, db); return code; };
    if (b->tree && !host_only) {
        int nc = 0;
        for (int i = 0; i < n; i++) nc += b->tree[i] == 2 && (b->cbf[i] & 6);
        if (nc) {
            db->h_chroma_cus = (uint32_t *)malloc(sizeof(uint32_t) * (size_t)nc);
            if (!db->h_chroma_cus) return fail(XGPU_ERR_OUT_OF_MEMORY);
            for (int i = 0; i < n; i++) if (b->tree[i] == 2 && (b->cbf[i] & 6)) db->h_chroma_cus[db->n_chroma_cus++] = (uint32_t)i;
        }
    }
    bool coef_pinned = host_only && b->n_coef != 0;
    if (const int rc = B.acquire_block(db, L, coef_pinned)) return fail(rc);
    if (coef_pinned) L.payload[SEG_COEF] = 0;
    BT("block");
    void *const hs = db->h_stage = db->blk.h_stage;
    B.copy_sliced(L.at<uint8_t>(hs, SEG_OWNER), S.own.data(), L.payload[SEG_OWNER]);
    B.fill_records(L, hs);
    B.fill_work_items(L.at<TbWave>(hs, SEG_WAVES));
    B.fill_items_and_copies(L, hs);
    uint8_t *const dbase = db->blk.d_base;
    db->d_cus = L.at<CuRec>(dbase, SEG_CUS); db->d_ctu_start = L.at<uint32_t>(dbase, SEG_CTU); db->d_tbs = L.at<TbRec>(dbase, SEG_TBS);
    db->d_waves = L.at<TbWave>(dbase, SEG_WAVES); db->d_intra = L.at<IntraRec>(dbase, SEG_INTRA); db->d_intra_deps = L.at<uint32_t>(dbase, SEG_DEPS);
    db->d_aff_items = L.at<AffItem>(dbase, SEG_AFF); db->d_cpmv = L.at<int16_t>(dbase, SEG_CPMV);
    db->d_dmvr_items = L.at<DmvrItem>(dbase, SEG_DMVR); db->d_dmvr_mv = L.at<int16_t>(dbase, SEG_DMV); db->d_owner = L.at<uint32_t>(dbase, SEG_OWNER);
    db->d_inter_items = L.at<InterItem>(dbase, SEG_IITEM); db->d_inter_work = L.at<uint32_t>(dbase, SEG_IWORK);
    db->d_coef = L.at<int16_t>(dbase, SEG_COEF); db->d_resid = L.at<int16_t>(dbase, SEG_RESID); db->d_intra_done = L.at<uint32_t>(dbase, SEG_DONE);
    BT("stage filled");
    if (layout) *layout = L;
    if (host_only) { *out = db; return XGPU_OK; }
    const hipError_t e = B.upload(db, L, coef_pinned);
    if (e != hipSuccess) { snprintf(c->err, sizeof(c->err), "batch upload: %s", hipGetErrorString(e)); return fail(XGPU_ERR_UNEXPECTED); }
    BT("uploads queued");
    *out = db; return XGPU_OK;
}
}
int xgpu_batch_create(xgpu_ctx *c, const xgpu_cu_batch *b, xgpu_dbatch **out) { return batch_build(c, b, out, false, NULL); }

int xgpu_test_build_batch(const xgpu_seq_params *sp, const xgpu_cu_batch *b, int threads, uint64_t digest[XGPU_TEST_BUILD_DIGESTS], int info[XGPU_BATCH_INFO_COUNT], double *ms)
{
    if (!sp || !b || !digest || threads < 1 || threads > 64) return XGPU_ERR_INVALID_ARGUMENT;
    if (sp->width <= 0 || sp->height <= 0 || (sp->width & 7) || (sp->height & 7) || sp->log2_ctu < 5 || sp->log2_ctu > 7) return XGPU_ERR_INVALID_ARGUMENT;
    xgpu_ctx *c = new xgpu_ctx();
    c->sp = *sp; c->sp.chroma_qp_table[0] = c->sp.chroma_qp_table[1] = NULL;
    c->builder_threads = threads; c->err[0] = 0;
    c->stream = c->up_stream = c->down_stream = c->side_stream = 0;
    ctx_geometry(c);
    xgpu_dbatch *db = NULL;
    StageLayout L;
    const auto t0 = std::chrono::steady_clock::now();
    const int rc = batch_build(c, b, &db, true, &L);
    if (ms) *ms = std::chrono::duration<double, std::milli>(std::chrono::steady_clock::now() - t0).count();
    if (rc == XGPU_OK) {
        static const Seg order[] = { SEG_CUS, SEG_CTU, SEG_TBS, SEG_WAVES, SEG_INTRA, SEG_DEPS, SEG_AFF, SEG_CPMV, SEG_DMVR, SEG_OWNER, SEG_COEF, SEG_IITEM, SEG_IWORK };
        for (int k = 0; k < XGPU_TEST_BUILD_DIGESTS; k++) {
            uint64_t h = 1469598103934665603ull;
            if (k < (int)(sizeof(order) / sizeof(order[0]))) { const uint8_t *p = L.at<uint8_t>(db->h_stage, order[k]); for (size_t i = 0; i < L.payload[order[k]]; i++) { h ^= p[i]; h *= 1099511628211ull; } }
            digest[k] = h;
        }
        if (info) batch_info_fill(db, info);
        xgpu_batch_destroy(c, db);
    }
    delete c;
    return rc;
}

void block_free(BatchBlock &blk)
{
    for (void *p : { (void *)blk.d_base, (void *)blk.d_chroma }) if (p) (void)hipFree(p);
    if (blk.h_stage) (void)hipHostFree(blk.h_stage);
    for (hipEvent_t e : { blk.uploaded, blk.done, blk.itdq_done }) if (e) (void)hipEventDestroy(e);
    memset(&blk, 0, sizeof(blk));
}

void xgpu_batch_destroy(xgpu_ctx *c, xgpu_dbatch *db)
{
    if (!db) return;
    if (db->host_only) { delete db; return; }
    if (db->h_chroma_cus) {
        if (db->blk.uploaded) (void)hipEventSynchronize(db->blk.uploaded);
        free(db->h_chroma_cus);
        db->h_chroma_cus = NULL;
    }
    if (db->blk.d_base && db->blk.h_stage && db->blk.uploaded && db->blk.done && db->blk.itdq_done && c) {
        if (db->prepared == 1) (void)hipStreamWaitEvent(c->stream, db->blk.itdq_done, 0);
        if (db->used || db->prepared) (void)hipEventRecord(db->blk.done, c->stream);
        std::lock_guard<std::mutex> g(c->pool_mu); c->pool.push_back(db->blk);
    }
    else {
        if (c && c->stream) (void)hipStreamSynchronize(c->stream);
        block_free(db->blk);
    }
    delete db;
}
int xgpu_set_builder_threads(xgpu_ctx *c, int n)
{
    ARGCHK(c, c != NULL); ARGCHK(c, n >= 1 && n <= 64);
    c->builder_threads = n;
    return XGPU_OK;
}
int xgpu_batch_info(xgpu_ctx *c, const xgpu_dbatch *db, int info[XGPU_BATCH_INFO_COUNT])
{
    ARGCHK(c, c != NULL); ARGCHK(c, db != NULL && info != NULL);
    batch_info_fill(db, info);
    return XGPU_OK;
}
int xgpu_batch_wait_upload(xgpu_ctx *c, xgpu_dbatch *db)
{
    ARGCHK(c, c != NULL); ARGCHK(c, db != NULL);
    HIPCHK(c, hipEventSynchronize(db->blk.uploaded));
    return XGPU_OK;
}
```

xevd_amd/csrc/xgpu_host.h:

```cpp
#pragma once
#include <math.h>
#include <stdlib.h>
#include <algorithm>
#include <atomic>
#include "xgpu_internal.h"

#define HIPCHK(c, expr)                                                                                         \
    do {                                                                                                        \
        hipError_t e_ = (expr);                                                                                 \
        if (e_ != hipSuccess) {                                                                                 \
            snprintf((c)->err, sizeof((c)->err), "%s:%d %s -> %s", __FILE__, __LINE__, #expr, hipGetErrorString(e_)); \
            return XGPU_ERR_UNEXPECTED;                                                                         \
        }                                                                                                       \
    } while (0)
#define ARGCHK(c, cond)                                                                                         \
    do {                                                                                                        \
        if (!(cond)) {                                                                                          \
            if (c) snprintf((c)->err, sizeof((c)->err), "%s:%d invalid argument: %s", __FILE__, __LINE__, #cond); \
            return XGPU_ERR_INVALID_ARGUMENT;                                                                   \
        }                                                                                                       \
    } while (0)


static inline int align_up(int v, int a) { return (v + a - 1) / a * a; }
static inline void ctx_geometry(xgpu_ctx *c)
{
    const int w = c->sp.width, h = c->sp.height, ctu = 1 << c->sp.log2_ctu;
    c->w_scu = w >> 2; c->h_scu = h >> 2; c->w_ctu = (w + ctu - 1) / ctu; c->h_ctu = (h + ctu - 1) / ctu;
    c->s_l = align_up(XGPU_MARGIN_L + w + XGPU_PAD_L, 64); c->s_c = align_up(XGPU_MARGIN_C + (w >> 1) + XGPU_PAD_C, 64);
    c->rows_l = h + 2 * XGPU_PAD_L; c->rows_c = (h >> 1) + 2 * XGPU_PAD_C;
    c->off_u = (size_t)c->s_l * c->rows_l; c->off_v = c->off_u + (size_t)c->s_c * c->rows_c;
    c->pic_elems = c->off_v + (size_t)c->s_c * c->rows_c + 64;
}
static inline bool valid_pic(const xgpu_ctx *c, int pic) { return pic >= 0 && pic + 1 < (int)c->pics.size() && c->pics[pic + 1].used; }
static inline DevPic &dpic(xgpu_ctx *c, int pic) { return c->pics[pic + 1]; }
static inline bool addb_alf_fused(const xgpu_ctx *c) { return c->fp.deblock_on && c->sp.tool_addb && c->fp.alf_on && !c->split_addb_alf; }

void time_begin(xgpu_ctx *c, int k, hipEvent_t *a, hipEvent_t *b);
void time_end(xgpu_ctx *c, int k, hipEvent_t a, hipEvent_t b);
#define TIMED(c, k, stmt)                      \
    do {                                       \
        hipEvent_t ta_ = 0, tb_ = 0;           \
        time_begin(c, k, &ta_, &tb_);          \
        stmt;                                  \
        time_end(c, k, ta_, tb_);              \
    } while (0)

__attribute__((visibility("hidden"))) int check_dra(xgpu_ctx *c, const xgpu_dra_luts *dra);
__attribute__((visibility("hidden"))) int upload_dra(xgpu_ctx *c, const xgpu_dra_luts *dra);

inline bool tile_mask(const xgpu_ctx *c, const xgpu_tile_grid *g, TileMask &m)
{
    memset(&m, 0, sizeof(m));
    if (!g) return true;
    if (g->n_cols < 1 || g->n_cols > XGPU_MAX_TILE_COLS || g->n_rows < 1 || g->n_rows > XGPU_MAX_TILE_ROWS || c->w_ctu > 256 || c->h_ctu > 256) return false;
    if (g->col_bd[0] != 0 || g->row_bd[0] != 0 || g->col_bd[g->n_cols] != c->w_ctu || g->row_bd[g->n_rows] != c->h_ctu) return false;
    for (int i = 0; i < g->n_cols; i++) if (g->col_bd[i + 1] <= g->col_bd[i]) return false;
    for (int j = 0; j < g->n_rows; j++) if (g->row_bd[j + 1] <= g->row_bd[j]) return false;
    for (int i = 1; i < g->n_cols; i++) m.vb[g->col_bd[i] >> 5] |= 1u << (g->col_bd[i] & 31);
    for (int j = 1; j < g->n_rows; j++) m.hb[g->row_bd[j] >> 5] |= 1u << (g->row_bd[j] & 31);
    return true;
}

static inline int plan_htdf_idx(const xgpu_cu_batch *b, uint32_t j)
{
    const int hqp = b->htdf_slice_qp;
    const bool intra = b->pred_mode[j] == XGPU_MODE_INTRA;
    if (hqp <= 17 || (b->tree && b->tree[j] == 2) || b->pred_mode[j] == XGPU_MODE_IBC || !((b->cbf[j] & 1) || intra)) return -1;
    const int w = 1 << b->log2w[j], h = 1 << b->log2h[j], mn = std::min(w, h), mx = std::max(w, h);
    if (w * h < 64 || mx >= 128 || (!intra && mn >= 32)) return -1;
    const int qp = hqp - ((intra && w == h && mn >= 32) ? 8 : 0);
    return std::min(std::max((qp - 20 + 4) >> 3, 0), 4);
}
static inline bool plan_is_node(const xgpu_cu_batch *b, uint32_t j) { return b->pred_mode[j] == XGPU_MODE_INTRA || b->pred_mode[j] == XGPU_MODE_IBC || plan_htdf_idx(b, j) >= 0; }
struct IntraPlan {
    std::vector<IntraRec> recs; std::vector<uint32_t> deps; bool has_ibc, has_htdf, has_right;
    int n_levels, n_level1, n_level1_small, n_heads;
    void reset() { recs.clear(); deps.clear(); n_levels = n_level1 = n_level1_small = n_heads = 0; has_ibc = has_htdf = has_right = false; }
};
struct PlanOut { std::vector<uint32_t> deps; bool ibc = false, htdf = false, right = false, bad = false; };
struct BuilderScratch {
    WorkPool pool;
    IntraPlan plan;
    std::vector<uint32_t> own, tile_cu, inter_items, inter_work, nodes;
    std::vector<uint8_t>  tile_any, host_stage;
    std::vector<uint32_t> owner_own, luma_owner, deps, succ, pos, nfirst;
    std::vector<int> level; std::vector<IntraRec> recs; std::vector<PlanOut> outs; std::vector<int32_t> rec_of_cu; std::vector<uint8_t> member;
};
__attribute__((visibility("hidden"))) bool build_intra_plan(xgpu_ctx *c, const xgpu_cu_batch *b, BuilderScratch &S, const uint32_t *final_owner, int nthr);
__attribute__((visibility("hidden"))) void block_free(BatchBlock &blk);
```

xevd_amd/csrc/xgpu_internal.h:

```cpp
#pragma once
#include <hip/hip_runtime.h>
#include <stdint.h>
#include <stdio.h>
#include <string.h>
#include <condition_variable>
#include <functional>
#include <mutex>
#include <thread>
#include <vector>
#include "../../include/xevd_hip.h"

#define XGPU_MARGIN_L 192
#define XGPU_MARGIN_C 128

struct DevPic {
    int16_t *base;
    int16_t *y, *u, *v;
    int      s_l, s_c;
    int      used;
};

struct __attribute__((aligned(16))) CuRec {
    uint16_t x, y;
    uint8_t  log2w, log2h;
    uint8_t  pred_mode;
    uint8_t  cbf;
    int8_t   refi[2];
    uint8_t  qp_map;
    uint8_t  map_cbf;
    uint32_t coef_off;
    int16_t  mv[2][2];
    uint8_t  qp[3];
    uint8_t  ipm[2];
    uint8_t  ats_inter;
    uint8_t  affine;
    uint8_t  dmvr;
};
static_assert(sizeof(CuRec) == 32, "CuRec must be 32 bytes");

struct __attribute__((aligned(16))) ScuRec {
    uint32_t scu;
    int8_t   refi[2];
    uint16_t ats_inter;
    int16_t  mv[2][2];
};
static_assert(sizeof(ScuRec) == 16, "ScuRec must be 16 bytes");
#define SCU_EDGE_L (1u << 8)
#define SCU_EDGE_T (1u << 9)
#define SCU_NOCH_L (1u << 10)
#define SCU_NOCH_T (1u << 11)
#define SCU_RANK(idx)  (((uint32_t)(idx) & 0xFFu) | ((((uint32_t)(idx) >> 8) & 7u) << 12))
#define SCU_RANK_OF(m) ((int)(((m) & 0xFFu) | (((m) >> 4) & 0x700u)))
#define CU_NOCH_L 0x40
#define CU_NOCH_T 0x80

struct TbRec {
    uint32_t off;
    uint8_t  log2w, log2h, qp;
    uint8_t  log2s;
};
#define TR_DCT2 0
#define TR_DST7 1
#define TR_DCT8 2
struct TbWave {
    uint32_t first;
    uint16_t count;
    uint8_t  log2w, log2h;
    uint8_t  tr_v, tr_h;
    uint8_t  pad[2];
};

#define XGPU_WORK_REGION 0x100u
#define XGPU_INTER_STRIP 16
struct __attribute__((aligned(16))) InterItem { uint32_t pos, cu, pad[2]; CuRec rec; };
static_assert(sizeof(InterItem) == 48, "InterItem must be 48 bytes");
struct RefEntry { const int16_t *y, *u, *v; int poc; int pad; };

struct InterArgs {
    int16_t *cur_y, *cur_u, *cur_v;
    int      s_l, s_c;
    int      pic_w, pic_h;
    int      bd_l, bd_c;
    int      admvp;
    const uint32_t  *work;
    const InterItem *items;
    int      n_work;
    int      regions_x, strip_entries, full_entries;
    uint32_t magic_strip, magic_last;
    const CuRec    *cus;
    const int16_t  *resid;
    ScuRec  *maps;
    int      w_scu;
    const uint32_t *owner;
    int      n_cu;
    int      cur_poc;
    int      dmvr_to_map;
    RefEntry refp[XGPU_MAX_REFS][2];
};

struct DmvrItem { uint32_t cu; uint8_t sx, sy; uint16_t pad; };
struct DmvrArgs {
    int16_t *cur_y, *cur_u, *cur_v;
    int      s_l, s_c;
    int      pic_w, pic_h;
    int      bd_l, bd_c;
    int      admvp, cur_poc;
    const CuRec    *cus;
    const DmvrItem *items;
    int      n_items;
    const int16_t  *resid;
    int16_t *out_mv;
    ScuRec  *maps;
    int      w_scu, refined_to_map;
    int      force_scalar;
    RefEntry refp[XGPU_MAX_REFS][2];
};

struct AffItem { uint32_t cu, aff; uint16_t tx, ty; uint32_t pad; };
static_assert(sizeof(AffItem) == 16, "AffItem must be 16 bytes");
struct AffineArgs {
    int16_t *cur_y, *cur_u, *cur_v;
    int      s_l, s_c;
    int      pic_w, pic_h;
    int      bd_l, bd_c;
    int      admvp;
    const CuRec   *cus;
    const int16_t *cpmv;
    const AffItem *items;
    int      n_eif, n_sub;
    const int16_t *resid;
    ScuRec  *maps;
    int      w_scu;
    RefEntry refp[XGPU_MAX_REFS][2];
};

struct __attribute__((aligned(16))) IntraRec {
    uint32_t cu;
    uint32_t flags;
    uint64_t up, le;
    uint32_t dep_first, dep_count;
    uint16_t x, y;
    uint8_t  log2w, log2h, cbf, pad0;
    uint8_t  ipm[2], pad1[2];
    uint32_t coef_off;
};
static_assert(sizeof(IntraRec) == 48, "IntraRec must be 48 bytes");
struct IntraArgs {
    int16_t *cur_y, *cur_u, *cur_v;
    int      s_l, s_c;
    int      bd_l, bd_c;
    const CuRec    *cus;
    const IntraRec *list;
    const uint32_t *deps;
    const int16_t  *resid;
    uint32_t *done;
    uint32_t  epoch, ticket_base;
    int       n_intra;
    int       first, count;
    int       n_small;
};

struct ItdqArgs {
    const int16_t *coef;
    int16_t       *resid;
    const TbRec   *tbs;
    const TbWave  *waves;
    int            n_waves;
    int            bd;
    int            iqt;
};

struct TileMask {
    uint32_t vb[8], hb[8];
    __host__ __device__ bool col_start(int ctu_x) const { return (vb[ctu_x >> 5] >> (ctu_x & 31)) & 1; }
    __host__ __device__ bool row_start(int ctu_y) const { return (hb[ctu_y >> 5] >> (ctu_y & 31)) & 1; }
    __host__ __device__ static int tile_first(const uint32_t *m, int i)
    {
        for (int w = i >> 5; w >= 0; w--) {
            uint32_t v = m[w];
            if (w == (i >> 5)) v &= 0xFFFFFFFFu >> (31 - (i & 31));
            if (v) return (w << 5) + 31 - __builtin_clz(v);
        }
        return 0;
    }
    __host__ __device__ static int tile_end(const uint32_t *m, int i, int n)
    {
        for (int w = (i + 1) >> 5; w < 8; w++) {
            uint32_t v = m[w];
            if (w == ((i + 1) >> 5)) v &= 0xFFFFFFFFu << ((i + 1) & 31);
            if (v) { const int e = (w << 5) + __builtin_ctz(v); return e < n ? e : n; }
        }
        return n;
    }
};

struct DbkArgs {
    int      s_l, s_c;
    int      pic_w, pic_h, w_scu, h_scu;
    int      bd_l, bd_c;
    int      ctu_sh;
    TileMask no_filter;
    const ScuRec *maps;
    uint8_t  st[3][4][64];
};

#define ADDB_LDS_TABLE_BYTES (52 + 52 + 260 + XGPU_MAX_REFS * 2 + 192)
#define ADDB_LDS_TABLE_DWORDS ((ADDB_LDS_TABLE_BYTES + 3) / 4)
struct AddbArgs {
    int      s_l, s_c;
    int      w_scu, h_scu;
    int      bd_l, bd_c, log2_ctu;
    int      alpha_off, beta_off, qp_u_off, qp_v_off;
    TileMask no_filter;
    const ScuRec *maps;
    int8_t   chroma_qp[2 * 96];
    uint8_t  pic_id[XGPU_MAX_REFS * 2];
    uint32_t lds_tables[ADDB_LDS_TABLE_DWORDS];
};

#define ALF_CTB_BITS 8704
struct AlfArgs {
    int      s_l, s_c, pic_w, pic_h, bd, log2_ctu, w_ctu, across_tiles;
    TileMask tiles;
    uint32_t magic_tiles_x;
    int      multi_tile;
    int      pad;
    int      enable[3];
    const uint8_t *ctb_flag;
    int      ctb_in_args;
    uint32_t ctb_bits[ALF_CTB_BITS / 32];
    uint32_t ctab[25 * 4][8];
    uint32_t cchroma[4];
};

struct BatchBlock { uint8_t *d_base; size_t d_cap; void *h_stage; size_t h_cap; hipEvent_t uploaded, done, itdq_done;
                    uint32_t *d_chroma; size_t chroma_cap; };

struct xgpu_dbatch {
    BatchBlock blk;
    int        n_cu, n_ctu, n_tb, n_waves;
    size_t     n_coef;
    CuRec     *d_cus;
    uint32_t  *d_ctu_start;
    uint32_t  *d_owner;
    InterItem *d_inter_items;
    uint32_t  *d_inter_work;
    int        n_inter_work;
    int16_t   *d_coef, *d_resid;
    TbRec     *d_tbs;
    TbWave    *d_waves;
    DmvrItem  *d_dmvr_items;
    int16_t   *d_dmvr_mv;
    int        n_dmvr;
    AffItem   *d_aff_items;
    int16_t   *d_cpmv;
    int        n_aff_eif, n_aff_sub;
    IntraRec  *d_intra;
    uint32_t  *d_intra_deps;
    uint32_t  *d_intra_done;
    int        has_ibc, has_htdf;
    int        order_rl;
    int        has_right;
    TileMask   tile_starts;
    int        tiles_across;
    int        n_intra_l1_small;
    int        n_intra, n_levels, n_intra_deps, n_intra_l1, n_intra_heads;
    uint32_t   intra_epoch, intra_tickets;
    void      *h_stage;
    int        host_only;
    size_t     stage_bytes;
    int        prepared;
    int        upload_waited;
    int        used;
    uint32_t  *h_chroma_cus, *d_chroma_cus;
    int        n_chroma_cus;
};

struct ScaleTabs { size_t off_first[4], off_count[4], off_w[4]; int stride[4]; int capy, capc; };
struct ScaleAxisTab { size_t first, count, w; int stride; };
struct xgpu_ctx {
    xgpu_seq_params sp;
    int8_t          chroma_qp[2][96];
    hipStream_t     stream;
    hipStream_t     up_stream, down_stream;
    hipStream_t     side_stream;
    hipEvent_t      after_inter;
    int             have_after_inter;
    std::mutex      pool_mu;
    struct HostRange { uint8_t *p; size_t n; };
    std::vector<HostRange> pinned;
    int             w_scu, h_scu, w_ctu, h_ctu;
    int             s_l, s_c, rows_l, rows_c;
    size_t          pic_elems, off_u, off_v;
    std::vector<DevPic> pics;
    ScuRec         *d_maps;
    uint8_t        *d_ctb_flag;
    std::vector<BatchBlock> pool;
    uint8_t        *d_out[2];
    uint8_t        *d_md5;
    hipEvent_t      md5_ready;
    size_t          out_caps[2];
    hipEvent_t      out_ready[2], out_done[2];
    int             out_busy[2], out_next;
    int32_t        *d_dra;
    float          *d_cm;
    xgpu_colour_tables_t *cm_tab;
    xgpu_colour_transform cm_key;
    int             cm_bd;
    uint8_t        *sc_tab;
    size_t          sc_tab_cap;
    int             sc_key[6];
    ScaleTabs       sc_host;
    uint16_t       *sc_mid;
    size_t          sc_mid_cap;
    unsigned long long *cmp_part;
    size_t          cmp_part_cap;
    uint8_t        *stats_blk;
    int             stats_lin_tc, stats_lin_bd;
    uint8_t        *rs_blk;
    size_t          rs_blk_cap;
    int             rs_key[7], rs_capy, rs_capc;
    uint8_t        *roi_blk;
    size_t          roi_blk_cap;
    uint8_t        *lad_blk;
    size_t          lad_blk_cap;
    std::vector<int> lad_key;
    std::vector<uint8_t> lad_host;
    std::vector<uint8_t> lad_sent;
    std::vector<ScaleAxisTab> lad_tabs;
    int             lad_cap;
    hipEvent_t      odev_ev[2];
    xgpu_frame_params fp;
    int             have_frame;
    int             side_pic;
    TileMask        no_dbk;
    hipEvent_t      fork_ev, join_ev;
    int             builder_threads;
    int             pad_done;
    int             where;
    int             order_rl;
    int             itdq_pair_min;
    int             intra_small_min;
    int             addb_scalar;
    int             dmvr_scalar;
    int             addb_pending, split_addb_alf;
    AddbArgs        addb_args;
    int             timing;
    struct Ev { hipEvent_t a, b; int k; };
    std::vector<Ev> ev_pending;
    std::vector<hipEvent_t> ev_pool;
    double          t_ms[XGPU_K_COUNT];
    long long       t_n[XGPU_K_COUNT];
    char            err[256];
};

class WorkPool {
public:
    ~WorkPool() { { std::lock_guard<std::mutex> g(mu); stop = true; } cv.notify_all(); for (std::thread &t : th) t.join(); }
    template <class F> void run(int n, F &&f)
    {
        if (n <= 1) { f(0); return; }
        while ((int)th.size() < n - 1) { const int idx = (int)th.size(); th.emplace_back([this, idx]() { worker(idx); }); }
        const std::function<void(int)> fn = [&f](int k) { f(k); };
        { std::lock_guard<std::mutex> g(mu); job = &fn; want = n - 1; left = n - 1; gen++; }
        cv.notify_all();
        f(0);
        std::unique_lock<std::mutex> g(mu);
        done_cv.wait(g, [this]() { return left == 0; });
        job = nullptr;
    }
private:
    void worker(int idx)
    {
        uint64_t seen = 0;
        for (;;) {
            const std::function<void(int)> *fn = nullptr;
            {
                std::unique_lock<std::mutex> g(mu);
                cv.wait(g, [&]() { return stop || gen != seen; });
                if (stop) return;
                seen = gen;
                if (idx < want) fn = job;
            }
            if (!fn) continue;
            (*fn)(idx + 1);
            std::lock_guard<std::mutex> g(mu);
            if (--left == 0) done_cv.notify_one();
        }
    }
    std::vector<std::thread> th;
    std::mutex mu;
    std::condition_variable cv, done_cv;
    const std::function<void(int)> *job = nullptr;
    int want = 0, left = 0;
    uint64_t gen = 0;
    bool stop = false;
};

void launch_itdq(xgpu_ctx *c, const ItdqArgs &a, hipStream_t s);
void launch_itdq_pairs(xgpu_ctx *c, const ItdqArgs &a, hipStream_t s);
void launch_inter(xgpu_ctx *c, const InterArgs &a);
void launch_test_recon(xgpu_ctx *c, const int16_t *coef, const int16_t *pred, int is_coef, int cuw, int cuh, int16_t *rec, int s_rec, int bd);
void launch_test_dbk(xgpu_ctx *c, int16_t *buf, int16_t *buf_v, int st, int st_v, int stride, int bd, int hor, int chroma);
void launch_intra(xgpu_ctx *c, const IntraArgs &a, bool dep, bool ibc, bool htdf, const ItdqArgs *next, bool right = false);
int  intra_chunk(bool with_itdq);
void launch_affine(xgpu_ctx *c, const AffineArgs &a, hipStream_t s);
void launch_dmvr(xgpu_ctx *c, const DmvrArgs &a, hipStream_t s);
void launch_dbk(xgpu_ctx *c, const DbkArgs &a, int dir, const DevPic &src, const DevPic &dst, bool order_rl = false);
void upload_transform_tables(const int *tm, const int16_t *ats, hipStream_t s);
int  itdq_group_size(int log2w, int log2h);
void launch_addb_fused(xgpu_ctx *c, const AddbArgs &a, const DevPic &src, const DevPic &dst);
void launch_alf(xgpu_ctx *c, const AlfArgs &a, const AddbArgs *deblock, const DevPic &src, const DevPic &dst);
void launch_pad(xgpu_ctx *c, const DevPic &p);
void launch_copy_bw(xgpu_ctx *c, const void *src, void *dst, size_t bytes);
void launch_output(xgpu_ctx *c, const DevPic &pic, const int32_t *d_dra, int out_bd, int crop_l, int crop_r, int crop_t, int crop_b, uint8_t *d_dst, bool raw16 = false,
                   hipStream_t s = nullptr);
struct RgbOutArgs {
    const int16_t *y, *u, *v;
    int      sy, sc;
    int      w, h, cw, ch;
    uint8_t *dst;
    size_t   pitch, plane;
    int      aligned;
    int      bgr;
    int      coef[5], shift;
// ... 224 lines not shown
```

xevd_amd/csrc/xgpu_launch.hip:

```cpp
#include "xgpu_host.h"
#include "addb_filter.h"

static const uint8_t k_df_st[4][52] = {
    { 0,0,0,0,0,0,0,0,0,0,0,0,0,0,0,0,0,0,1,1,1,1,1,1,1,1,1,2,2,2,2,2,3,3,3,4,4,4,5,5,6,6,7,8,9,10,11,12,12,12,12,12 },
    { 0,0,0,0,0,0,0,0,0,0,0,0,0,0,0,0,0,0,0,0,0,0,0,0,0,0,0,1,1,1,1,1,2,2,2,3,3,3,4,4,5,5,6,7,8, 9,10,11,11,11,11,11 },
    { 0,0,0,0,0,0,0,0,0,0,0,0,0,0,0,0,0,0,0,0,0,0,0,0,0,0,0,0,0,0,0,0,1,1,1,2,2,2,3,3,4,4,5,6,7, 8, 9,10,10,10,10,10 },
    { 0 },
};

static ItdqArgs itdq_args(const xgpu_ctx *c, const xgpu_dbatch *db)
{
    ItdqArgs ia;
    ia.coef = db->d_coef; ia.resid = db->d_resid; ia.tbs = db->d_tbs; ia.waves = db->d_waves; ia.n_waves = db->n_waves;
    ia.bd = c->sp.bit_depth_luma;
    ia.iqt = c->sp.tool_iqt;
    return ia;
}

int xgpu_batch_prepare(xgpu_ctx *c, xgpu_dbatch *db)
{
    ARGCHK(c, c != NULL); ARGCHK(c, db != NULL);
    if (db->prepared) return XGPU_OK;
    HIPCHK(c, hipStreamWaitEvent(c->side_stream, db->blk.uploaded, 0));
    if (c->have_after_inter) HIPCHK(c, hipStreamWaitEvent(c->side_stream, c->after_inter, 0));
    const ItdqArgs ia = itdq_args(c, db);
    launch_itdq(c, ia, c->side_stream);
    HIPCHK(c, hipGetLastError());
    HIPCHK(c, hipEventRecord(db->blk.itdq_done, c->side_stream));
    db->prepared = 1;
    return XGPU_OK;
}

int xgpu_batch_recon(xgpu_ctx *c, xgpu_dbatch *db) { return xgpu_batch_recon_ahead(c, db, NULL); }

int xgpu_batch_recon_ahead(xgpu_ctx *c, xgpu_dbatch *db, xgpu_dbatch *next)
{
    ARGCHK(c, c != NULL); ARGCHK(c, db != NULL); ARGCHK(c, c->have_frame); ARGCHK(c, next != db);
    if (!db->upload_waited) HIPCHK(c, hipStreamWaitEvent(c->stream, db->blk.uploaded, 0));
    db->upload_waited = 0;
    db->used = 1;
    if (next && next->prepared) next = NULL;
    const bool ahead = next != NULL;
    bool next_waited = false;
    auto wait_next = [&]() -> int {
        if (next && !next_waited) { HIPCHK(c, hipStreamWaitEvent(c->stream, next->blk.uploaded, 0)); next_waited = true; }
        return XGPU_OK;
    };
    if (db->tiles_across) memset(&c->no_dbk, 0, sizeof(c->no_dbk)); else c->no_dbk = db->tile_starts;
    if (db->prepared == 2) {
        db->prepared = 0;
    } else if (db->prepared) {
        HIPCHK(c, hipStreamWaitEvent(c->stream, db->blk.itdq_done, 0));
        db->prepared = 0;
    } else {
        const ItdqArgs ia = itdq_args(c, db);
        TIMED(c, XGPU_K_ITDQ, launch_itdq(c, ia, c->stream));
    }

    InterArgs a;
    memset(&a, 0, sizeof(a));
    c->where = (addb_alf_fused(c) ? 1 : (c->fp.deblock_on ? (c->sp.tool_addb ? 1 : 2) : 0) + (c->fp.alf_on ? 1 : 0)) & 1;
    DevPic &cur = c->where ? c->pics[0] : dpic(c, c->fp.pic);
    a.cur_y = cur.y; a.cur_u = cur.u; a.cur_v = cur.v;
    a.s_l = c->s_l; a.s_c = c->s_c; a.pic_w = c->sp.width; a.pic_h = c->sp.height;
    a.bd_l = c->sp.bit_depth_luma; a.bd_c = c->sp.bit_depth_chroma;
    a.admvp = c->sp.tool_admvp ? 1 : 0;
    a.work = db->d_inter_work; a.items = db->d_inter_items; a.n_work = db->n_inter_work;
    {
        const int regions_x = (c->sp.width + 63) >> 6, regions_y = (c->sp.height + 63) >> 6;
        a.regions_x = regions_x; a.strip_entries = XGPU_INTER_STRIP * regions_y; a.full_entries = (regions_x / XGPU_INTER_STRIP) * a.strip_entries;
        a.magic_strip = (uint32_t)((1ull << 32) / (uint64_t)a.strip_entries) + 1u;
        a.magic_last = (regions_x % XGPU_INTER_STRIP) > 1 ? (uint32_t)((1ull << 32) / (uint64_t)(regions_x % XGPU_INTER_STRIP)) + 1u : 0u;
    }
    a.cus = db->d_cus; a.resid = db->d_resid;
    a.maps = c->d_maps; a.w_scu = c->w_scu; a.owner = db->d_owner; a.n_cu = db->n_cu; a.cur_poc = c->fp.poc;
    c->order_rl |= db->order_rl;
    for (int l = 0; l < 2; l++)
        for (int i = 0; i < XGPU_MAX_REFS; i++) {
            const DevPic &rp = i < c->fp.num_refp[l] ? dpic(c, c->fp.refp_pic[i][l]) : dpic(c, c->fp.pic);
            a.refp[i][l].y = rp.y; a.refp[i][l].u = rp.u; a.refp[i][l].v = rp.v;
            a.refp[i][l].poc = i < c->fp.num_refp[l] ? c->fp.refp_poc[i][l] : 0;
        }
    static const bool serial_knob = getenv("XEVD_HIP_TOOLS_SERIAL") != NULL;
    const bool beside = !c->timing && !serial_knob && (db->n_dmvr || db->n_aff_eif + db->n_aff_sub);
    hipStream_t tool_stream = c->stream;
    a.dmvr_to_map = c->sp.tool_addb ? 0 : 1;
    if (beside) {
        HIPCHK(c, hipEventRecord(c->fork_ev, c->stream));
        HIPCHK(c, hipStreamWaitEvent(c->side_stream, c->fork_ev, 0));
        tool_stream = c->side_stream;
    }
    TIMED(c, XGPU_K_INTER, launch_inter(c, a));
    if (!ahead) HIPCHK(c, hipEventRecord(c->after_inter, c->stream));
    c->have_after_inter = 1;
    if (db->n_dmvr) {
        DmvrArgs d;
        memset(&d, 0, sizeof(d));
        d.cur_y = cur.y; d.cur_u = cur.u; d.cur_v = cur.v; d.s_l = c->s_l; d.s_c = c->s_c; d.pic_w = c->sp.width; d.pic_h = c->sp.height;
        d.bd_l = c->sp.bit_depth_luma; d.bd_c = c->sp.bit_depth_chroma; d.admvp = a.admvp; d.cur_poc = c->fp.poc;
        d.cus = db->d_cus; d.items = db->d_dmvr_items; d.n_items = db->n_dmvr; d.resid = db->d_resid; d.out_mv = db->d_dmvr_mv; d.maps = c->d_maps; d.w_scu = c->w_scu; d.refined_to_map = c->sp.tool_addb ? 0 : 1; d.force_scalar = c->dmvr_scalar;
        memcpy(d.refp, a.refp, sizeof(d.refp));
        TIMED(c, XGPU_K_DMVR, launch_dmvr(c, d, tool_stream));
    }
    if (db->n_aff_eif + db->n_aff_sub) {
        AffineArgs f;
        memset(&f, 0, sizeof(f));
        f.cur_y = cur.y; f.cur_u = cur.u; f.cur_v = cur.v; f.s_l = c->s_l; f.s_c = c->s_c; f.pic_w = c->sp.width; f.pic_h = c->sp.height;
        f.bd_l = c->sp.bit_depth_luma; f.bd_c = c->sp.bit_depth_chroma; f.admvp = a.admvp;
        f.cus = db->d_cus; f.cpmv = db->d_cpmv; f.items = db->d_aff_items; f.n_eif = db->n_aff_eif; f.n_sub = db->n_aff_sub;
        f.resid = db->d_resid; f.maps = c->d_maps; f.w_scu = c->w_scu;
        memcpy(f.refp, a.refp, sizeof(f.refp));
        TIMED(c, XGPU_K_AFFINE, launch_affine(c, f, tool_stream));
    }
    if (beside) {
        HIPCHK(c, hipEventRecord(c->join_ev, c->side_stream));
        HIPCHK(c, hipStreamWaitEvent(c->stream, c->join_ev, 0));
    }
    if (db->n_intra) {
        IntraArgs ta;
        ta.cur_y = cur.y; ta.cur_u = cur.u; ta.cur_v = cur.v; ta.s_l = c->s_l; ta.s_c = c->s_c; ta.bd_l = c->sp.bit_depth_luma; ta.bd_c = c->sp.bit_depth_chroma;
        ta.cus = db->d_cus; ta.list = db->d_intra; ta.deps = db->d_intra_deps; ta.resid = db->d_resid;
        ta.done = db->d_intra_done; ta.n_intra = db->n_intra;
        ta.epoch = ++db->intra_epoch;
        ta.ticket_base = db->intra_tickets;
        const int n_dep = db->n_intra_heads - db->n_intra_l1;
        {
            ItdqArgs na;
            const bool ride = next && n_dep > 0 && !c->timing && !db->has_htdf && (na = itdq_args(c, next), na.n_waves > 0);
            if (ride) { const int rc = wait_next(); if (rc != XGPU_OK) return rc; }
            TIMED(c, XGPU_K_INTRA, {
                ta.first = 0; ta.count = db->n_intra_l1; ta.n_small = db->n_intra_l1_small;
                if (ta.count) launch_intra(c, ta, false, db->has_ibc != 0, db->has_htdf != 0, NULL, db->has_right != 0);
                ta.first = db->n_intra_l1; ta.count = n_dep; ta.n_small = 0;
                if (n_dep) {
                    launch_intra(c, ta, true, db->has_ibc != 0, db->has_htdf != 0, ride ? &na : NULL, db->has_right != 0);
                    const int chunk = intra_chunk(ride);
                    db->intra_tickets += (uint32_t)((ta.count + chunk - 1) / chunk);
                    if (ride) { next->upload_waited = 1; next->prepared = 2; next->used = 1; next = NULL; }
                }
            });
        }
    }
    if (next) {
        const int rc = wait_next();
        if (rc != XGPU_OK) return rc;
        const ItdqArgs na = itdq_args(c, next);
        TIMED(c, XGPU_K_ITDQ, launch_itdq(c, na, c->stream));
        next->upload_waited = 1; next->prepared = 2; next->used = 1;
    }
    HIPCHK(c, hipGetLastError());
    return XGPU_OK;
}

int xgpu_batch_dmvr_mvs(xgpu_ctx *c, xgpu_dbatch *db, int16_t *mv, int n)
{
    ARGCHK(c, c != NULL); ARGCHK(c, db != NULL && n >= 0);
// ... 142 lines not shown
```

Measured before the change: 3471 frames/s.

## Reorder inter work and filter tiles to shrink kernel tail imbalance

```diff
diff --git a/include/xevd_hip.h b/include/xevd_hip.h
--- a/include/xevd_hip.h
+++ b/include/xevd_hip.h
@@ -404,6 +404,7 @@
 int xgpu_test_batch_resid(xgpu_ctx *ctx, xgpu_dbatch *db, int16_t *resid);
 #define XGPU_TEST_BUILD_DIGESTS 13
 int xgpu_test_build_batch(const xgpu_seq_params *sp, const xgpu_cu_batch *b, int threads, uint64_t digest[XGPU_TEST_BUILD_DIGESTS], int info[XGPU_BATCH_INFO_COUNT], double *ms);
+int xgpu_test_launch_order(const xgpu_seq_params *sp, const xgpu_cu_batch *b, int light_last, int border_first, uint32_t *inter_region, uint32_t *inter_work, uint32_t *filter_tile, int cap, int n[2]);
 int xgpu_test_itdq(xgpu_ctx *ctx, int16_t *coef, int n_blocks, int log2w, int log2h, const uint8_t *qp, int bit_depth);
 int xgpu_test_itdq_ex(xgpu_ctx *ctx, int16_t *coef, int n_blocks, int log2w, int log2h, const uint8_t *qp, int bit_depth, int tr_v, int tr_h, int log2s);
 int xgpu_test_itdq_pairs(xgpu_ctx *ctx, int16_t *coef, int n_blocks, int log2w, int log2h, const uint8_t *qp, int bit_depth, int tr_v, int tr_h, int log2s);
diff --git a/xevd_amd/abi.py b/xevd_amd/abi.py
--- a/xevd_amd/abi.py
+++ b/xevd_amd/abi.py
@@ -806,6 +806,7 @@
     "xgpu_test_mc_c": (C.c_int, [C.c_void_p, C.c_void_p] + [C.c_int] * 8 + [C.c_void_p] + [C.c_int] * 3),
     "xgpu_test_batch_resid": (C.c_int, [C.c_void_p, C.c_void_p, C.c_void_p]),
     "xgpu_test_build_batch": (C.c_int, [C.c_void_p, C.c_void_p, C.c_int, C.POINTER(C.c_uint64), C.POINTER(C.c_int), C.POINTER(C.c_double)]),
+    "xgpu_test_launch_order": (C.c_int, [C.c_void_p, C.c_void_p, C.c_int, C.c_int, C.POINTER(C.c_uint32), C.POINTER(C.c_uint32), C.POINTER(C.c_uint32), C.c_int, C.POINTER(C.c_int)]),
     "xgpu_test_recon": (C.c_int, [C.c_void_p, C.c_void_p, C.c_void_p] + [C.c_int] * 4 + [C.c_void_p, C.c_int]),
     "xgpu_test_dbk": (C.c_int, [C.c_void_p, C.c_void_p] + [C.c_int] * 7),
     "xgpu_test_dbk_chroma": (C.c_int, [C.c_void_p, C.c_void_p, C.c_void_p] + [C.c_int] * 8),
diff --git a/xevd_amd/csrc/k_alf.hip b/xevd_amd/csrc/k_alf.hip
--- a/xevd_amd/csrc/k_alf.hip
+++ b/xevd_amd/csrc/k_alf.hip
@@ -131,16 +131,13 @@
     int16_t (*b_row)[2][64] = (int16_t (*)[2][64])l_y, (*b_col)[2][64] = (int16_t (*)[2][64])(l_y + 3 * 2 * 64);
     static_assert(2 * 3 * 2 * 64 <= LROWS * LSTR, "the border arrays fit into the staged luma tile");
 
-    const int tiles_x = (a.pic_w + 63) >> 6, n_tiles = tiles_x * ((a.pic_h + 63) >> 6);
-    const int per_xcd = gridDim.x >> 3, xcd = blockIdx.x & 7, seq = blockIdx.x >> 3;
-    const int tile = xcd * per_xcd + (xcd >= 4 ? per_xcd - 1 - seq : seq);
-    if (tile >= n_tiles) return;
-    const int ty = a.magic_tiles_x ? (int)__umulhi((uint32_t)tile, a.magic_tiles_x) : tile, tx = tile - ty * tiles_x;
+    int tx, ty;
+    if (!filter_tile_at(a.order, (int)blockIdx.x, tx, ty)) return;
     const int tx0 = tx << 6, ty0 = ty << 6;
     const int t = threadIdx.x;
 #ifdef XGPU_ALF_TRACE
     unsigned long long atr_prev = __builtin_amdgcn_s_memtime();
-    const bool atr_on = (t & 63) == 0 && tile % 61 == 7;
+    const bool atr_on = (t & 63) == 0 && (ty * a.order.tiles_x + tx) % 61 == 7;
     if (atr_on) atomicAdd(&g_alf_trace[15], 1ull);
 #endif
     CtuRect k, kc;
@@ -654,19 +651,34 @@
     alf_kernel<false>(a, nullptr, sy_, su_, sv_, dy_, du_, dv_);
 }
 
+#ifdef XGPU_TAIL_TRACE
+__device__ unsigned long long g_tail_filter[XGPU_TAIL_CAP][3];
+extern "C" int xgpu_test_filter_tail(unsigned long long *out, int n_waves)
+{
+    if (n_waves < 0 || n_waves > XGPU_TAIL_CAP) return -1;
+    return hipMemcpyFromSymbol(out, HIP_SYMBOL(g_tail_filter), sizeof(unsigned long long) * 3 * (size_t)n_waves) == hipSuccess ? 0 : -1;
+}
+#endif
 template <bool PK>
 __global__ __launch_bounds__(256) __attribute__((amdgpu_waves_per_eu(XGPU_ALF_WAVES, XGPU_ALF_WAVES))) void k_addb_alf(const AlfArgs a, const AddbArgs d, const int16_t *__restrict__ sy_, const int16_t *__restrict__ su_,
                                                   const int16_t *__restrict__ sv_, int16_t *__restrict__ dy_, int16_t *__restrict__ du_, int16_t *__restrict__ dv_)
 {
+#ifdef XGPU_TAIL_TRACE
+    const unsigned long long t0 = tail_now();
+#endif
     alf_kernel<true, PK>(a, &d, sy_, su_, sv_, dy_, du_, dv_);
+#ifdef XGPU_TAIL_TRACE
+    int tx, ty;
+    const bool any = filter_tile_at(a.order, (int)blockIdx.x, tx, ty);
+    tail_store(g_tail_filter, t0, !any ? 3u : (tx == 0 || ty == 0 || tx == a.order.tiles_x - 1 || ty == a.order.tiles_y - 1) ? 1u : 0u);
+#endif
 }
 
 void launch_alf(xgpu_ctx *c, const AlfArgs &a_, const AddbArgs *deblock, const DevPic &src, const DevPic &dst)
 {
     AlfArgs a = a_;
-    const int tiles = ((a.pic_w + 63) >> 6) * ((a.pic_h + 63) >> 6);
-    a.magic_tiles_x = a.pic_w > 64 ? (uint32_t)((1ull << 32) / (uint64_t)((a.pic_w + 63) >> 6)) + 1u : 0u;
-    const dim3 grid(((tiles + 7) >> 3) << 3);
+    filter_order_init(a.order, a.pic_w, a.pic_h, c->filter_border_first != 0);
+    const dim3 grid((unsigned)filter_order_grid(a.order));
     const bool scalar_knob = c->addb_scalar != 0;
     static const int lds_pad = getenv("XEVD_HIP_ALF_LDSPAD") ? atoi(getenv("XEVD_HIP_ALF_LDSPAD")) : 0;
     if (deblock && !scalar_knob && deblock->bd_l <= 10 && deblock->bd_c <= 10) hipLaunchKernelGGL(k_addb_alf<true>, grid, dim3(256), lds_pad, c->stream, a, *deblock, src.y, src.u, src.v, dst.y, dst.u, dst.v);
diff --git a/xevd_amd/csrc/k_inter.hip b/xevd_amd/csrc/k_inter.hip
--- a/xevd_amd/csrc/k_inter.hip
+++ b/xevd_amd/csrc/k_inter.hip
@@ -654,7 +654,6 @@
     return true;
 }
 
-__device__ __forceinline__ int xcd_slice(int block, int grid) { return (block & 7) * (grid >> 3) + (block >> 3); }
 
 __device__ __forceinline__ void store_scu(const InterArgs &a, int sx, int sy, const uint32_t pl[8], const uint32_t pu[2], const uint32_t pv[2])
 {
@@ -672,7 +671,6 @@
 #define ARG_LTAPS(a) ((const uint4 *)&k_luma_taps[(a).admvp][0][0])
 #define ARG_CTAPS(a) ((const uint2 *)&k_chroma_taps[(a).admvp][0][0])
 static_assert(sizeof(RefEntry) == 32, "a reference entry is two 16-byte halves");
-static_assert(XGPU_INTER_STRIP == 16, "the strip arithmetic below shifts by four");
 
 struct SplitTables { uint4 ref[XGPU_MAX_REFS * 2][2]; uint4 ltap[17]; uint2 ctap[33]; uint2 pad; };
 
@@ -681,24 +679,17 @@
     __shared__ __attribute__((aligned(16))) int16_t s_win[REG_SAMPLES];
     static_assert(4 * UNI_SAMPLES <= REG_SAMPLES, "the four waves' tile blocks fit into the region block");
     __shared__ SplitTables s_tab[4];
-    const int idx = xcd_slice(blockIdx.x, gridDim.x);
+    const int idx = inter_slot((int)blockIdx.x, (int)gridDim.x);
     if (idx >= a.n_work) return;
     const int t = threadIdx.x, lane = t & 63, wave = __builtin_amdgcn_readfirstlane(t >> 6);
 #ifdef XGPU_INTER_TRACE
     InterTrace tr = { __builtin_amdgcn_s_memtime(), 0, lane == 0 && (idx % 61) == 7 };
 #endif
-    int rx, ry;
-    if (idx < a.full_entries) {
-        const int s = (int)__umulhi((uint32_t)idx, a.magic_strip), r = idx - s * a.strip_entries;
-        ry = r >> 4; rx = (s << 4) + (r & 15);
-    } else {
-        const int r = idx - a.full_entries;
-        ry = a.magic_last ? (int)__umulhi((uint32_t)r, a.magic_last) : r; rx = (a.regions_x & ~15) + r - ry * (a.regions_x & 15);
-    }
-    const int sx = (rx << 4) + ((wave & 1) << 3) + (lane & 7), sy = (ry << 4) + ((wave >> 1) << 3) + (lane >> 3);
     const uint32_t kinds = a.work[idx];
     const uint4 *const item = (const uint4 *)&a.items[idx * 4 + wave];
     const uint4 e = item[0], i0 = item[1], i1 = item[2];
+    const int rx = __builtin_amdgcn_readfirstlane((int)(e.x & 0xFFFFu)), ry = __builtin_amdgcn_readfirstlane((int)(e.x >> 16));
+    const int sx = (rx << 4) + ((wave & 1) << 3) + (lane & 7), sy = (ry << 4) + ((wave >> 1) << 3) + (lane >> 3);
     const uint32_t own = (sx < (a.pic_w >> 2) && sy < (a.pic_h >> 2)) ? a.owner[sy * a.w_scu + sx] : OWNER_NONE;
     const LaneMap fm0 = { 0, 0 };
     uint32_t pl[8], pu[2], pv[2];
@@ -755,12 +746,29 @@
         TRACE_MARK(tr, 10);
     }
 }
+#ifdef XGPU_TAIL_TRACE
+__device__ unsigned long long g_tail_inter[XGPU_TAIL_CAP][3];
+extern "C" int xgpu_test_inter_tail(unsigned long long *out, int n_waves)
+{
+    if (n_waves < 0 || n_waves > XGPU_TAIL_CAP) return -1;
+    return hipMemcpyFromSymbol(out, HIP_SYMBOL(g_tail_inter), sizeof(unsigned long long) * 3 * (size_t)n_waves) == hipSuccess ? 0 : -1;
+}
+__global__ __launch_bounds__(256) void k_inter(const InterArgs a)
+{
+    const unsigned long long t0 = tail_now();
+    inter_fused_body(a);
+    const int idx = inter_slot((int)blockIdx.x, (int)gridDim.x);
+    const uint32_t kinds = idx < a.n_work ? a.work[idx] : 0u;
+    tail_store(g_tail_inter, t0, kinds == XGPU_WORK_REGION ? 0u : (kinds & 0xAAu) ? 2u : kinds ? 1u : 3u);
+}
+#else
 __global__ __launch_bounds__(256) void k_inter(const InterArgs a) { inter_fused_body(a); }
+#endif
 
 void launch_inter(xgpu_ctx *c, const InterArgs &a)
 {
     if (!a.n_work) return;
-    const dim3 grid((unsigned)(((a.n_work + 7) >> 3) << 3));
+    const dim3 grid((unsigned)inter_grid(a.n_work));
     hipLaunchKernelGGL(k_inter, grid, dim3(256), 0, c->stream, a);
 }
 
diff --git a/xevd_amd/csrc/xgpu_api.hip b/xevd_amd/csrc/xgpu_api.hip
--- a/xevd_amd/csrc/xgpu_api.hip
+++ b/xevd_amd/csrc/xgpu_api.hip
@@ -112,6 +112,7 @@
     c->fork_ev = c->join_ev = 0;
     c->itdq_pair_min = getenv("XEVD_HIP_ITDQ_PAIR_MIN") ? std::max(1, atoi(getenv("XEVD_HIP_ITDQ_PAIR_MIN"))) : 4096;
     c->intra_small_min = getenv("XEVD_HIP_INTRA_SMALL_MIN") ? std::max(1, atoi(getenv("XEVD_HIP_INTRA_SMALL_MIN"))) : 2048;
+    ctx_order_knobs(c);
     c->addb_scalar = getenv("XEVD_HIP_ADDB_SCALAR") != NULL;
     c->dmvr_scalar = getenv("XEVD_HIP_DMVR_SCALAR") != NULL;
     c->split_addb_alf = getenv("XEVD_HIP_SPLIT_ADDB_ALF") != NULL;
diff --git a/xevd_amd/csrc/xgpu_builder.hip b/xevd_amd/csrc/xgpu_builder.hip
--- a/xevd_amd/csrc/xgpu_builder.hip
+++ b/xevd_amd/csrc/xgpu_builder.hip
@@ -3,7 +3,7 @@
 #include "affine_model.h"
 
 namespace {
-enum Seg { SEG_CUS, SEG_CTU, SEG_TBS, SEG_WAVES, SEG_INTRA, SEG_DEPS, SEG_AFF, SEG_CPMV, SEG_DMVR, SEG_OWNER, SEG_IITEM, SEG_IWORK, SEG_COEF, SEG_RESID, SEG_DONE, SEG_DMV, SEG_COUNT };
+enum Seg { SEG_CUS, SEG_CTU, SEG_TBS, SEG_WAVES, SEG_INTRA, SEG_DEPS, SEG_AFF, SEG_CPMV, SEG_DMVR, SEG_OWNER, SEG_IITEM, SEG_IWORK, SEG_LITEM, SEG_LWORK, SEG_COEF, SEG_RESID, SEG_DONE, SEG_DMV, SEG_COUNT };
 struct StageLayout {
     size_t off[SEG_COUNT], alloc[SEG_COUNT], payload[SEG_COUNT], stage_bytes, d_need;
     template <class T> T *at(void *base, Seg s) const { return (T *)((uint8_t *)base + off[s]); }
@@ -176,12 +176,13 @@
                     }
             }
         });
-        inter_items.clear(); inter_work.clear();
+        inter_items.clear(); inter_work.clear(); S.inter_pos.clear();
         const int regions_x = (c->sp.width + 63) >> 6, regions_y = (c->sp.height + 63) >> 6;
         for (int s0 = 0; s0 < regions_x; s0 += XGPU_INTER_STRIP)
             for (int ry = 0; ry < regions_y; ry++)
                 for (int rx = s0; rx < std::min(s0 + XGPU_INTER_STRIP, regions_x); rx++) {
                     const int tx = rx * 2, ty = ry * 2;
+                    S.inter_pos.push_back((uint32_t)rx | ((uint32_t)ry << 16));
                     const bool whole = tx + 1 < tiles_x && ty + 1 < tiles_y;
                     const uint32_t o = tcu[(size_t)ty * tiles_x + tx];
                     if (whole && o != 0xFFFFFFFFu && tcu[(size_t)ty * tiles_x + tx + 1] == o && tcu[(size_t)(ty + 1) * tiles_x + tx] == o && tcu[(size_t)(ty + 1) * tiles_x + tx + 1] == o) {
@@ -203,6 +204,28 @@
                     inter_work.push_back(kinds);
                 }
     }
+    void inter_launch_order()
+    {
+        const int n_work = (int)S.inter_work.size(), G = (n_work + 7) >> 3, light_last = c->inter_light_last;
+        std::vector<uint32_t> &ord = S.inter_order; ord.resize((size_t)n_work);
+        for (int i = 0; i < n_work; i++) ord[(size_t)i] = (uint32_t)i;
+        if (!light_last) return;
+        const uint32_t *const work = S.inter_work.data();
+        auto weight = [work](uint32_t e) { const uint32_t k = work[e]; return k == XGPU_WORK_REGION ? 1 : (k & 0xAAu) ? 3 : k ? 2 : 0; };
+        for (int k0 = 0; k0 < n_work; k0 += G) {
+            const int k1 = std::min(k0 + G, n_work);
+            int left[4] = { 0, 0, 0, 0 }, want = (light_last < 0 || light_last > k1 - k0) ? k1 - k0 : light_last;
+            for (int i = k0; i < k1; i++) left[weight((uint32_t)i)]++;
+            for (int w = 0; w < 4; w++) { const int take = std::min(left[w], want); left[w] = take; want -= take; }
+            uint32_t *const o = ord.data() + k0;
+            int head = k1 - k0, tail[4];
+            for (int w = 0; w < 4; w++) head -= left[w];
+            for (int w = 3, at = head; w >= 0; w--) { tail[w] = at; at += left[w]; }
+            std::vector<uint8_t> &in_tail = S.tile_any; in_tail.assign((size_t)(k1 - k0), 0);
+            for (int i = k1 - 1; i >= k0; i--) { const int w = weight((uint32_t)i); if (left[w]) { left[w]--; in_tail[(size_t)(i - k0)] = 1; } }
+            for (int i = k0, h = 0; i < k1; i++) { if (in_tail[(size_t)(i - k0)]) o[tail[weight((uint32_t)i)]++] = (uint32_t)i; else o[h++] = (uint32_t)i; }
+        }
+    }
     bool probe_order_rl()
     {
         if (c->sp.tool_addb) return false;
@@ -338,12 +361,19 @@
     void fill_items_and_copies(const StageLayout &L, void *hs)
     {
         memcpy(L.at<uint8_t>(hs, SEG_CTU), b->ctu_cu_start, L.payload[SEG_CTU]);
-        InterItem *const it = L.at<InterItem>(hs, SEG_IITEM); const CuRec *const cus = L.at<CuRec>(hs, SEG_CUS);
-        const uint32_t *const ii = S.inter_items.data(); const size_t n_items = S.inter_items.size();
-        S.pool.run(nthr, [&, it, ii](int part) {
-            for (size_t k = n_items * (size_t)part / nthr; k < n_items * (size_t)(part + 1) / nthr; k++) {
-                if (ii[k] == 0xFFFFFFFFu) memset(&it[k], 0, sizeof(InterItem));
-                else { it[k].pos = 0; it[k].cu = ii[k]; it[k].pad[0] = it[k].pad[1] = 0; it[k].rec = cus[ii[k]]; }
+        InterItem *const it = L.at<InterItem>(hs, SEG_IITEM), *const lit = L.at<InterItem>(hs, SEG_LITEM); const CuRec *const cus = L.at<CuRec>(hs, SEG_CUS);
+        uint32_t *const lwork = L.at<uint32_t>(hs, SEG_LWORK);
+        const uint32_t *const ii = S.inter_items.data(), *const ord = S.inter_order.data(), *const pos = S.inter_pos.data(), *const work = S.inter_work.data();
+        const size_t n_work = S.inter_work.size();
+        S.pool.run(nthr, [&, it, lit, lwork, ii, ord, pos, work](int part) {
+            for (size_t p = n_work * (size_t)part / nthr; p < n_work * (size_t)(part + 1) / nthr; p++) {
+                const uint32_t e = ord[p];
+                lwork[p] = work[e];
+                for (size_t k = (size_t)e * 4, l = p * 4; k < (size_t)e * 4 + 4; k++, l++) {
+                    if (ii[k] == 0xFFFFFFFFu) memset(&it[k], 0, sizeof(InterItem));
+                    else { it[k].pos = 0; it[k].cu = ii[k]; it[k].pad[0] = it[k].pad[1] = 0; it[k].rec = cus[ii[k]]; }
+                    lit[l] = it[k]; lit[l].pos = pos[e];
+                }
             }
         });
         if (L.payload[SEG_IWORK]) memcpy(L.at<uint8_t>(hs, SEG_IWORK), S.inter_work.data(), L.payload[SEG_IWORK]);
@@ -354,7 +384,8 @@
     hipError_t upload(xgpu_dbatch *db, const StageLayout &L, bool coef_pinned)
     {
         uint8_t *const dbase = db->blk.d_base;
-        hipError_t e = hipMemcpyAsync(dbase, db->h_stage, coef_pinned ? L.off[SEG_COEF] : L.stage_bytes, hipMemcpyHostToDevice, c->up_stream);
+        const size_t first = L.off[SEG_CUS];
+        hipError_t e = hipMemcpyAsync(dbase + first, (const uint8_t *)db->h_stage + first, (coef_pinned ? L.off[SEG_COEF] : L.stage_bytes) - first, hipMemcpyHostToDevice, c->up_stream);
         if (e == hipSuccess && coef_pinned) e = hipMemcpyAsync(dbase + L.off[SEG_COEF], b->coef, sizeof(int16_t) * b->n_coef, hipMemcpyHostToDevice, c->up_stream);
         if (e == hipSuccess && db->n_chroma_cus) e = hipMemcpyAsync(db->d_chroma_cus, db->h_chroma_cus, sizeof(uint32_t) * (size_t)db->n_chroma_cus, hipMemcpyHostToDevice, c->up_stream);
         if (e == hipSuccess) e = hipMemsetAsync(db->d_intra_done, 0, L.alloc[SEG_DONE], c->up_stream);
@@ -391,6 +422,7 @@
     B.paint_owner_map();
     BT("owner map");
     B.inter_work_lists();
+    B.inter_launch_order();
     BT("inter lists");
     const bool order_rl = B.probe_order_rl();
     ARGCHK(c, B.intra_plan());
@@ -400,9 +432,9 @@
     memset(db, 0, sizeof(*db)); db->host_only = host_only ? 1 : 0;
     db->n_cu = n; db->n_ctu = b->n_ctu; db->n_tb = B.n_tb; db->n_waves = B.n_waves; db->n_coef = b->n_coef; db->n_intra = n_intra; db->n_intra_deps = n_deps; db->n_levels = plan.n_levels; db->n_intra_l1 = plan.n_level1; db->n_intra_l1_small = plan.n_level1_small; db->n_intra_heads = plan.n_heads; db->n_aff_eif = B.n_aff_eif; db->n_aff_sub = B.n_aff_sub; db->n_dmvr = B.n_dmvr; db->has_ibc = plan.has_ibc ? 1 : 0; db->has_htdf = plan.has_htdf ? 1 : 0; db->has_right = plan.has_right ? 1 : 0; db->order_rl = order_rl ? 1 : 0;
     db->tile_starts = tmask; db->tiles_across = b->tiles ? (b->tiles->loop_filter_across_tiles ? 1 : 0) : 1; db->n_inter_work = (int)S.inter_work.size();
-    const SegSize rows[] = { { SEG_CUS, sizeof(CuRec), (size_t)n, 1 }, { SEG_CTU, sizeof(uint32_t), (size_t)b->n_ctu + 1, 1 }, { SEG_TBS, sizeof(TbRec), (size_t)B.n_tb, 1 }, { SEG_WAVES, sizeof(TbWave), (size_t)B.n_waves, 1 },
+    const SegSize rows[] = { { SEG_IITEM, sizeof(InterItem), S.inter_items.size(), 1 }, { SEG_IWORK, sizeof(uint32_t), S.inter_work.size(), 1 }, { SEG_CUS, sizeof(CuRec), (size_t)n, 1 }, { SEG_CTU, sizeof(uint32_t), (size_t)b->n_ctu + 1, 1 }, { SEG_TBS, sizeof(TbRec), (size_t)B.n_tb, 1 }, { SEG_WAVES, sizeof(TbWave), (size_t)B.n_waves, 1 },
         { SEG_INTRA, sizeof(IntraRec), (size_t)n_intra, 1 }, { SEG_DEPS, sizeof(uint32_t), (size_t)n_deps, 1 }, { SEG_AFF, sizeof(AffItem), (size_t)(B.n_aff_eif + B.n_aff_sub), 1 }, { SEG_CPMV, sizeof(int16_t) * 12, (size_t)B.n_aff, 1 },
-        { SEG_DMVR, sizeof(DmvrItem), (size_t)B.n_dmvr, 1 }, { SEG_OWNER, sizeof(uint32_t), (size_t)c->w_scu * c->h_scu, 0 }, { SEG_IITEM, sizeof(InterItem), S.inter_items.size(), 1 }, { SEG_IWORK, sizeof(uint32_t), S.inter_work.size(), 1 },
+        { SEG_DMVR, sizeof(DmvrItem), (size_t)B.n_dmvr, 1 }, { SEG_OWNER, sizeof(uint32_t), (size_t)c->w_scu * c->h_scu, 0 }, { SEG_LITEM, sizeof(InterItem), S.inter_items.size(), 1 }, { SEG_LWORK, sizeof(uint32_t), S.inter_work.size(), 1 },
         { SEG_COEF, sizeof(int16_t), b->n_coef, 8 }, { SEG_RESID, sizeof(int16_t), b->n_coef, 8 }, { SEG_DONE, sizeof(uint32_t), (size_t)n_intra + 1, 1 }, { SEG_DMV, sizeof(int16_t) * 4, (size_t)B.n_dmvr, 1 } };
     StageLayout L; stage_layout(L, rows); db->stage_bytes = L.stage_bytes;
     auto fail = [&](int code) { xgpu_batch_destroy(c, db); return code; };
@@ -429,7 +461,7 @@
     db->d_waves = L.at<TbWave>(dbase, SEG_WAVES); db->d_intra = L.at<IntraRec>(dbase, SEG_INTRA); db->d_intra_deps = L.at<uint32_t>(dbase, SEG_DEPS);
     db->d_aff_items = L.at<AffItem>(dbase, SEG_AFF); db->d_cpmv = L.at<int16_t>(dbase, SEG_CPMV);
     db->d_dmvr_items = L.at<DmvrItem>(dbase, SEG_DMVR); db->d_dmvr_mv = L.at<int16_t>(dbase, SEG_DMV); db->d_owner = L.at<uint32_t>(dbase, SEG_OWNER);
-    db->d_inter_items = L.at<InterItem>(dbase, SEG_IITEM); db->d_inter_work = L.at<uint32_t>(dbase, SEG_IWORK);
+    db->d_inter_items = L.at<InterItem>(dbase, SEG_LITEM); db->d_inter_work = L.at<uint32_t>(dbase, SEG_LWORK);
     db->d_coef = L.at<int16_t>(dbase, SEG_COEF); db->d_resid = L.at<int16_t>(dbase, SEG_RESID); db->d_intra_done = L.at<uint32_t>(dbase, SEG_DONE);
     BT("stage filled");
     if (layout) *layout = L;
@@ -442,15 +474,22 @@
 }
 int xgpu_batch_create(xgpu_ctx *c, const xgpu_cu_batch *b, xgpu_dbatch **out) { return batch_build(c, b, out, false, NULL); }
 
-int xgpu_test_build_batch(const xgpu_seq_params *sp, const xgpu_cu_batch *b, int threads, uint64_t digest[XGPU_TEST_BUILD_DIGESTS], int info[XGPU_BATCH_INFO_COUNT], double *ms)
-{
-    if (!sp || !b || !digest || threads < 1 || threads > 64) return XGPU_ERR_INVALID_ARGUMENT;
-    if (sp->width <= 0 || sp->height <= 0 || (sp->width & 7) || (sp->height & 7) || sp->log2_ctu < 5 || sp->log2_ctu > 7) return XGPU_ERR_INVALID_ARGUMENT;
+static xgpu_ctx *deviceless_ctx(const xgpu_seq_params *sp, int threads)
+{
+    if (!sp || threads < 1 || threads > 64) return NULL;
+    if (sp->width <= 0 || sp->height <= 0 || (sp->width & 7) || (sp->height & 7) || sp->log2_ctu < 5 || sp->log2_ctu > 7) return NULL;
     xgpu_ctx *c = new xgpu_ctx();
     c->sp = *sp; c->sp.chroma_qp_table[0] = c->sp.chroma_qp_table[1] = NULL;
-    c->builder_threads = threads; c->err[0] = 0;
+    c->builder_threads = threads; c->err[0] = 0; ctx_order_knobs(c);
     c->stream = c->up_stream = c->down_stream = c->side_stream = 0;
     ctx_geometry(c);
+    return c;
+}
+int xgpu_test_build_batch(const xgpu_seq_params *sp, const xgpu_cu_batch *b, int threads, uint64_t digest[XGPU_TEST_BUILD_DIGESTS], int info[XGPU_BATCH_INFO_COUNT], double *ms)
+{
+    if (!b || !digest) return XGPU_ERR_INVALID_ARGUMENT;
+    xgpu_ctx *c = deviceless_ctx(sp, threads);
+    if (!c) return XGPU_ERR_INVALID_ARGUMENT;
     xgpu_dbatch *db = NULL;
     StageLayout L;
     const auto t0 = std::chrono::steady_clock::now();
@@ -470,6 +509,33 @@
     return rc;
 }
 
+int xgpu_test_launch_order(const xgpu_seq_params *sp, const xgpu_cu_batch *b, int light_last, int border_first, uint32_t *inter_region, uint32_t *inter_work, uint32_t *filter_tile, int cap, int n[2])
+{
+    if (!b || !inter_region || !inter_work || !filter_tile || !n || cap < 0) return XGPU_ERR_INVALID_ARGUMENT;
+    xgpu_ctx *c = deviceless_ctx(sp, 1);
+    if (!c) return XGPU_ERR_INVALID_ARGUMENT;
+    c->inter_light_last = light_last; c->filter_border_first = border_first ? 1 : 0;
+    xgpu_dbatch *db = NULL;
+    StageLayout L;
+    const int rc = batch_build(c, b, &db, true, &L);
+    if (rc == XGPU_OK) {
+        const int regions_x = (sp->width + 63) >> 6, n_work = db->n_inter_work;
+        const InterItem *const items = L.at<InterItem>(db->h_stage, SEG_LITEM); const uint32_t *const work = L.at<uint32_t>(db->h_stage, SEG_LWORK);
+        n[0] = inter_grid(n_work);
+        for (int p = 0; p < std::min(n[0], cap); p++) {
+            const int slot = inter_slot(p, n[0]);
+            inter_region[p] = slot < n_work ? (items[(size_t)slot * 4].pos >> 16) * (uint32_t)regions_x + (items[(size_t)slot * 4].pos & 0xFFFFu) : 0xFFFFFFFFu;
+            inter_work[p] = slot < n_work ? work[slot] : 0u;
+        }
+        FilterOrder fo; filter_order_init(fo, sp->width, sp->height, border_first != 0);
+        n[1] = filter_order_grid(fo);
+        for (int p = 0; p < std::min(n[1], cap); p++) { int tx, ty; filter_tile[p] = filter_tile_at(fo, p, tx, ty) ? (uint32_t)(ty * fo.tiles_x + tx) : 0xFFFFFFFFu; }
+        xgpu_batch_destroy(c, db);
+    }
+    delete c;
+    return rc;
+}
+
 void block_free(BatchBlock &blk)
 {
     for (void *p : { (void *)blk.d_base, (void *)blk.d_chroma }) if (p) (void)hipFree(p);
diff --git a/xevd_amd/csrc/xgpu_host.h b/xevd_amd/csrc/xgpu_host.h
--- a/xevd_amd/csrc/xgpu_host.h
+++ b/xevd_amd/csrc/xgpu_host.h
@@ -31,6 +31,12 @@
     c->rows_l = h + 2 * XGPU_PAD_L; c->rows_c = (h >> 1) + 2 * XGPU_PAD_C;
     c->off_u = (size_t)c->s_l * c->rows_l; c->off_v = c->off_u + (size_t)c->s_c * c->rows_c;
     c->pic_elems = c->off_v + (size_t)c->s_c * c->rows_c + 64;
+}
+static inline void ctx_order_knobs(xgpu_ctx *c)
+{
+    const char *io = getenv("XEVD_HIP_INTER_ORDER"), *fo = getenv("XEVD_HIP_FILTER_ORDER");
+    c->inter_light_last = io ? atoi(io) : XGPU_INTER_LIGHT_LAST;
+    c->filter_border_first = fo ? atoi(fo) != 0 : 1;
 }
 static inline bool valid_pic(const xgpu_ctx *c, int pic) { return pic >= 0 && pic + 1 < (int)c->pics.size() && c->pics[pic + 1].used; }
 static inline DevPic &dpic(xgpu_ctx *c, int pic) { return c->pics[pic + 1]; }
@@ -82,7 +88,7 @@
 struct BuilderScratch {
     WorkPool pool;
     IntraPlan plan;
-    std::vector<uint32_t> own, tile_cu, inter_items, inter_work, nodes;
+    std::vector<uint32_t> own, tile_cu, inter_items, inter_work, inter_pos, inter_order, nodes;
     std::vector<uint8_t>  tile_any, host_stage;
     std::vector<uint32_t> owner_own, luma_owner, deps, succ, pos, nfirst;
     std::vector<int> level; std::vector<IntraRec> recs; std::vector<PlanOut> outs; std::vector<int32_t> rec_of_cu; std::vector<uint8_t> member;
diff --git a/xevd_amd/csrc/xgpu_internal.h b/xevd_amd/csrc/xgpu_internal.h
--- a/xevd_amd/csrc/xgpu_internal.h
+++ b/xevd_amd/csrc/xgpu_internal.h
@@ -85,8 +85,6 @@
     const uint32_t  *work;
     const InterItem *items;
     int      n_work;
-    int      regions_x, strip_entries, full_entries;
-    uint32_t magic_strip, magic_last;
     const CuRec    *cus;
     const int16_t  *resid;
     ScuRec  *maps;
@@ -218,11 +216,69 @@
     uint32_t lds_tables[ADDB_LDS_TABLE_DWORDS];
 };
 
+struct FilterOrder { int tiles_x, tiles_y, n_tiles, n_border, per_xcd, border_first; uint32_t magic_x, magic_ix; };
+static inline uint32_t order_magic(int d) { return d > 1 ? (uint32_t)((1ull << 32) / (uint64_t)d) + 1u : 0u; }
+static inline void filter_order_init(FilterOrder &o, int pic_w, int pic_h, bool border_first)
+{
+    o.tiles_x = (pic_w + 63) >> 6; o.tiles_y = (pic_h + 63) >> 6; o.n_tiles = o.tiles_x * o.tiles_y;
+    const int iw = o.tiles_x > 2 ? o.tiles_x - 2 : 0, ih = o.tiles_y > 2 ? o.tiles_y - 2 : 0;
+    o.border_first = border_first ? 1 : 0;
+    o.n_border = border_first ? o.n_tiles - iw * ih : 0;
+    o.per_xcd = ((border_first ? iw * ih : o.n_tiles) + 7) >> 3;
+    o.magic_x = order_magic(o.tiles_x); o.magic_ix = order_magic(iw);
+}
+static inline int filter_order_grid(const FilterOrder &o) { return 8 * (((o.n_border + 7) >> 3) + o.per_xcd); }
+__host__ __device__ inline int order_quot(int n, uint32_t magic) { return magic ? (int)(((uint64_t)(uint32_t)n * magic) >> 32) : n; }
+__host__ __device__ inline bool filter_tile_at(const FilterOrder &o, int b, int &tx, int &ty)
+{
+    const int xcd = b & 7;
+    if (!o.border_first) {
+        const int seq = b >> 3, tile = xcd * o.per_xcd + (xcd >= 4 ? o.per_xcd - 1 - seq : seq);
+        if (tile >= o.n_tiles) return false;
+        ty = order_quot(tile, o.magic_x); tx = tile - ty * o.tiles_x;
+        return true;
+    }
+    if (b < o.n_border) {
+        int j = b;
+        if (j < o.tiles_x) { tx = j; ty = o.tiles_y - 1; return true; }
+        j -= o.tiles_x;
+        if (j < o.tiles_x) { tx = j; ty = 0; return true; }
+        j -= o.tiles_x;
+        if (o.tiles_x > 1) { tx = (j & 1) ? o.tiles_x - 1 : 0; ty = 1 + (j >> 1); }
+        else { tx = 0; ty = 1 + j; }
+        return true;
+    }
+    const int seq = (b >> 3) - ((o.n_border + 7 - xcd) >> 3), tile = xcd * o.per_xcd + seq, iw = o.tiles_x - 2;
+    if (seq >= o.per_xcd || tile >= iw * (o.tiles_y - 2)) return false;
+    const int iy = order_quot(tile, o.magic_ix);
+    tx = 1 + tile - iy * iw; ty = 1 + iy;
+    return true;
+}
+
+#ifndef XGPU_INTER_LIGHT_LAST
+#define XGPU_INTER_LIGHT_LAST 128
+#endif
+__host__ __device__ inline int inter_slot(int block, int grid) { return (block & 7) * (grid >> 3) + (block >> 3); }
+static inline int inter_grid(int n_work) { return ((n_work + 7) >> 3) << 3; }
+
+#ifdef XGPU_TAIL_TRACE
+#define XGPU_TAIL_CAP (4 * 8704)
+__device__ __forceinline__ unsigned long long tail_now() { const unsigned long long t = wall_clock64(); __builtin_amdgcn_s_waitcnt(0xC07F); return t; }
+__device__ __forceinline__ void tail_store(unsigned long long (*buf)[3], unsigned long long t0, uint32_t cls)
+{
+    const unsigned w = blockIdx.x * 4 + (threadIdx.x >> 6);
+    if ((threadIdx.x & 63) == 0 && w < XGPU_TAIL_CAP) {
+        const uint32_t xcc = (uint32_t)__builtin_amdgcn_s_getreg((3 << 11) | 20) & 15u;
+        buf[w][0] = t0; buf[w][1] = wall_clock64(); buf[w][2] = cls | (xcc << 8);
+    }
+}
+#endif
+
 #define ALF_CTB_BITS 8704
 struct AlfArgs {
     int      s_l, s_c, pic_w, pic_h, bd, log2_ctu, w_ctu, across_tiles;
     TileMask tiles;
-    uint32_t magic_tiles_x;
+    FilterOrder order;
     int      multi_tile;
     int      pad;
     int      enable[3];
@@ -341,6 +397,8 @@
     int             order_rl;
     int             itdq_pair_min;
     int             intra_small_min;
+    int             inter_light_last;
+    int             filter_border_first;
     int             addb_scalar;
     int             dmvr_scalar;
     int             addb_pending, split_addb_alf;
diff --git a/xevd_amd/csrc/xgpu_launch.hip b/xevd_amd/csrc/xgpu_launch.hip
--- a/xevd_amd/csrc/xgpu_launch.hip
+++ b/xevd_amd/csrc/xgpu_launch.hip
@@ -66,12 +66,6 @@
     a.bd_l = c->sp.bit_depth_luma; a.bd_c = c->sp.bit_depth_chroma;
     a.admvp = c->sp.tool_admvp ? 1 : 0;
     a.work = db->d_inter_work; a.items = db->d_inter_items; a.n_work = db->n_inter_work;
-    {
-        const int regions_x = (c->sp.width + 63) >> 6, regions_y = (c->sp.height + 63) >> 6;
-        a.regions_x = regions_x; a.strip_entries = XGPU_INTER_STRIP * regions_y; a.full_entries = (regions_x / XGPU_INTER_STRIP) * a.strip_entries;
-        a.magic_strip = (uint32_t)((1ull << 32) / (uint64_t)a.strip_entries) + 1u;
-        a.magic_last = (regions_x % XGPU_INTER_STRIP) > 1 ? (uint32_t)((1ull << 32) / (uint64_t)(regions_x % XGPU_INTER_STRIP)) + 1u : 0u;
-    }
     a.cus = db->d_cus; a.resid = db->d_resid;
     a.maps = c->d_maps; a.w_scu = c->w_scu; a.owner = db->d_owner; a.n_cu = db->n_cu; a.cur_poc = c->fp.poc;
     c->order_rl |= db->order_rl;
```

Result: no change. 3536 frames/s, median of 6 (+1.9%).
